# ViV99/slam-experiments

Measured on AMD Instinct MI355X. Metric: descriptor pairs/sec BF-Hamming knn=2 @64kx64k, higher is better.
Workload: dtype u32

## Files before the change

### include/slamhip.h

```cpp
#ifndef SLAMHIP_H
#define SLAMHIP_H

#include <stdint.h>

#ifdef __cplusplus
extern "C" {
#endif

typedef struct slam_ctx slam_ctx;

#define SLAM_API __attribute__((visibility("default")))

enum slam_status {
    SLAM_OK = 0,
    SLAM_ERR_INVALID = -1,
    SLAM_ERR_HIP = -2,
    SLAM_ERR_NO_DEVICE = -3,
    SLAM_ERR_RCCL = -4,
    SLAM_ERR_STATE = -5,
    SLAM_ERR_BUSY = -6
};

#define SLAM_DESC_BYTES 32
#define SLAM_MAX_TRAIN_PER_PASS (1 << 23)
#define SLAM_NO_MATCH_IDX (-1)
#define SLAM_NO_MATCH_DIST 2147483647

SLAM_API const char* slam_last_error(void);
SLAM_API const char* slam_version(void);
SLAM_API int slam_device_count(int* count);
SLAM_API int slam_ctx_create(int device, slam_ctx** out);
SLAM_API int slam_ctx_destroy(slam_ctx* ctx);
SLAM_API int slam_ctx_device(slam_ctx* ctx, int* device);
SLAM_API int slam_sync(slam_ctx* ctx);
SLAM_API int slam_ctx_block_bytes(slam_ctx* ctx, int64_t* h_bytes, int count);
SLAM_API int slam_ctx_block_fill(slam_ctx* ctx, int block, int byte);

SLAM_API int slam_malloc(slam_ctx* ctx, uint64_t bytes, void** d_ptr);
SLAM_API int slam_free(slam_ctx* ctx, void* d_ptr);
SLAM_API int slam_memset(slam_ctx* ctx, void* d_ptr, int value, uint64_t bytes);
SLAM_API int slam_copy(slam_ctx* ctx, void* d_dst, const void* d_src, uint64_t bytes);
SLAM_API int slam_upload(slam_ctx* ctx, void* d_dst, const void* h_src, uint64_t bytes);
SLAM_API int slam_download(slam_ctx* ctx, void* h_dst, const void* d_src, uint64_t bytes);

SLAM_API int slam_timer_start(slam_ctx* ctx);
SLAM_API int slam_timer_stop(slam_ctx* ctx, float* ms);
SLAM_API int slam_prof_enable(slam_ctx* ctx, int on);
SLAM_API int slam_prof_read(slam_ctx* ctx, int64_t* launches, double* total_ms);

SLAM_API int slam_bf_knn2_u256(slam_ctx* ctx, const void* d_query, int64_t N,
                      const void* d_train, int64_t M, int64_t train_base,
                      int32_t* d_idx, int32_t* d_dist);

#define SLAM_BF_BATCH_MAX 32
typedef struct slam_bf_search {
    const void* d_query;
    int64_t N;
    const void* d_train;
    int64_t M;
    int64_t train_base;
    int32_t* d_idx;
    int32_t* d_dist;
} slam_bf_search;
SLAM_API int slam_bf_knn2_batch_u256(slam_ctx* ctx, int64_t B, const slam_bf_search* h_searches);

SLAM_API int slam_bf_merge_top2(slam_ctx* ctx, const int32_t* d_idx_parts,
                       const int32_t* d_dist_parts, int64_t G, int64_t N,
                       int32_t* d_idx, int32_t* d_dist);

SLAM_API int slam_bf_knn2_u256_host(slam_ctx* ctx, const uint8_t* h_query, int64_t N,
                           const uint8_t* h_train, int64_t M,
                           int32_t* h_idx, int32_t* h_dist);

#define SLAM_BF_KNN_MAX 32
SLAM_API int slam_bf_knn_u256(slam_ctx* ctx, const void* d_query, int64_t N, const void* d_train, int64_t M,
                              int64_t train_base, int K, int32_t* d_idx, int32_t* d_dist);
SLAM_API int slam_bf_knn_u256_host(slam_ctx* ctx, const uint8_t* h_query, int64_t N, const uint8_t* h_train, int64_t M,
                                   int K, int32_t* h_idx, int32_t* h_dist);
SLAM_API int slam_bf_merge_topk(slam_ctx* ctx, const int32_t* d_idx_parts, const int32_t* d_dist_parts, int64_t G,
                                int64_t N, int K, int32_t* d_idx, int32_t* d_dist);
SLAM_API int slam_bf_topk_plan_describe(int num_cu, int64_t N, int64_t M, int K, int32_t* h_plan);

SLAM_API int slam_bf_radius_u256(slam_ctx* ctx, const void* d_query, int64_t N, const void* d_train, int64_t M,
                                 float max_distance, int64_t train_base, int64_t* d_offsets, int64_t capacity,
                                 int32_t* d_idx, int32_t* d_dist, int64_t* h_total);
SLAM_API int slam_bf_radius_u256_host(slam_ctx* ctx, const uint8_t* h_query, int64_t N, const uint8_t* h_train, int64_t M,
                                      float max_distance, int64_t* h_offsets, int64_t capacity, int32_t* h_idx,
                                      int32_t* h_dist, int64_t* h_total);
SLAM_API int slam_bf_radius_threshold(float max_distance);
SLAM_API int slam_bf_radius_plan_describe(int num_cu, int64_t N, int64_t M, int32_t* h_plan);

SLAM_API int slam_bf_window_knn_u256(slam_ctx* ctx, const void* d_query, int64_t N, const void* d_train, int64_t M,
                                     const float* d_query_xy, const float* d_train_xy, const float* d_radius, float radius,
                                     int k, int64_t cells, int32_t* d_idx, int32_t* d_dist);
SLAM_API int slam_bf_window_knn_u256_host(slam_ctx* ctx, const uint8_t* h_query, int64_t N, const uint8_t* h_train, int64_t M,
                                          const float* h_query_xy, const float* h_train_xy, const float* h_radius,
                                          float radius, int k, int64_t cells, int32_t* h_idx, int32_t* h_dist);
SLAM_API int slam_bf_window_plan_describe(int num_cu, int64_t N, int64_t M, int64_t cells, int64_t* h_plan);

#define SLAM_BF_KNOBS 10
SLAM_API int slam_bf_set_tuning(slam_ctx* ctx, const int32_t* h_knobs, int count);
SLAM_API int slam_bf_plan_info(slam_ctx* ctx, int64_t N, int64_t M, int32_t* h_plan);
SLAM_API int slam_bf_plan_describe(int num_cu, const int32_t* h_knobs, int count, int64_t N, int64_t M, int64_t qb_all,
                                   int rows_on_host, int32_t* h_plan, int32_t* h_tbl, int64_t tbl_cap, int64_t* tbl_len);
SLAM_API int slam_bf_set_engine(slam_ctx* ctx, int engine);
SLAM_API int slam_bf_mx_plan_describe(int num_cu, int64_t N, int64_t M, int32_t* h_plan, int32_t* h_tbl, int64_t tbl_cap,
                                      int64_t* tbl_len);
SLAM_API int slam_bf_mx_tile_describe(int engine, int64_t N, int64_t M, int32_t* h_tile);
SLAM_API int slam_bf_reset_state(slam_ctx* ctx);
SLAM_API int slam_bf_state_dirty(slam_ctx* ctx, int64_t* h_words);

SLAM_API int slam_bf_knn2_select_u256(slam_ctx* ctx, const void* d_query, int64_t N, const void* d_train, int64_t M,
                                      int64_t train_base, int32_t* d_idx, int32_t* d_dist, int mode, double param,
                                      uint8_t* d_keep, int64_t* h_count);

SLAM_API int slam_bf_match_filter(slam_ctx* ctx, const int32_t* d_idx, const int32_t* d_dist,
                         int64_t N, int mode, double param,
                         uint8_t* d_keep, int64_t* h_count, int32_t* h_min_dist);

SLAM_API int slam_bf_cross_check(slam_ctx* ctx, const int32_t* d_fwd_idx, const int32_t* d_fwd_dist, int64_t N,
                        const int32_t* d_rev_idx, int64_t M, int32_t* d_out_idx, int32_t* d_out_dist,
                        int64_t* h_count);

SLAM_API int slam_bf_split_index(slam_ctx* ctx, const int32_t* d_global_idx, int64_t count, const int32_t* d_offsets,
                                 int64_t images, int32_t* d_img_idx, int32_t* d_train_idx);

SLAM_API int slam_reproj_rj_f64(slam_ctx* ctx, const double* d_poses, int64_t K,
                       const double* d_points, int64_t L,
                       const int32_t* d_obs_pose, const int32_t* d_obs_point,
                       const double* d_meas, int64_t O,
                       double fx, double fy, double cx, double cy,
                       double* d_e, double* d_Jpose, double* d_Jpoint);

SLAM_API int slam_index_errors(slam_ctx* ctx, int64_t* count);

SLAM_API int slam_pose_normal_eq_f64(slam_ctx* ctx, const double* d_pose,
                            const double* d_points, const double* d_meas,
                            const uint8_t* d_active, int64_t O,
                            double fx, double fy, double cx, double cy,
                            double huber_delta,
                            double* d_H, double* d_b, double* d_chi2);

SLAM_API int slam_pose_optimize_f64(slam_ctx* ctx, const double* d_pose_in, const double* d_points,
                                    const double* d_meas, int64_t O, double fx, double fy, double cx, double cy,
                                    int rounds, int iterations, double chi2_threshold, double huber_delta,
                                    double* d_pose_out, uint8_t* d_inlier, double* d_chi2, int32_t* d_stats);

SLAM_API int slam_pose_optimize_batch_f64(slam_ctx* ctx, int64_t B, const double* d_pose_in, const double* d_points,
                                          const double* d_meas, const int32_t* d_offsets, int64_t O_total, double fx,
                                          double fy, double cx, double cy, int rounds, int iterations,
                                          double chi2_threshold, double huber_delta, double* d_pose_out,
                                          uint8_t* d_inlier, double* d_chi2, int32_t* d_stats);


SLAM_API int slam_tv_fivepoint_f64(slam_ctx* ctx, int64_t S, const double* d_x1, const double* d_x2, double* d_E,
                                   int32_t* d_nroots);

SLAM_API int slam_tv_essential_ransac_f64(slam_ctx* ctx, int64_t B, const int32_t* d_offsets, const double* d_px1,
                                          const double* d_px2, int64_t M, double fx, double fy, double cx, double cy,
                                          int H, double threshold_px, uint64_t seed, double* d_E, uint8_t* d_inlier,
                                          int32_t* d_stats);

SLAM_API int slam_tv_recover_pose_f64(slam_ctx* ctx, int64_t B, const int32_t* d_offsets, const double* d_px1,
                                      const double* d_px2, int64_t M, double fx, double fy, double cx, double cy,
                                      const double* d_E, const uint8_t* d_inlier_in, double distance_thresh,
                                      double* d_pose, uint8_t* d_inlier_out, int32_t* d_stats);

SLAM_API int slam_tv_triangulate_f64(slam_ctx* ctx, int64_t N, const double* d_P1, const double* d_P2,
                                     const double* d_x1, const double* d_x2, double* d_X, double* d_w);


SLAM_API int slam_pnp_p3p_f64(slam_ctx* ctx, int64_t S, const double* d_X, const double* d_x, double* d_pose,
                              int32_t* d_nsol);

SLAM_API int slam_pnp_ransac_f64(slam_ctx* ctx, int64_t B, const int32_t* d_offsets, const double* d_X,
                                 const double* d_px, int64_t M, double fx, double fy, double cx, double cy, int H,
                                 double threshold_px, uint64_t seed, double* d_pose, uint8_t* d_inlier,
                                 int32_t* d_stats);


SLAM_API int slam_hg_fourpoint_f64(slam_ctx* ctx, int64_t S, const double* d_p1, const double* d_p2, double* d_H,
                                   int32_t* d_ok);

SLAM_API int slam_hg_ransac_f64(slam_ctx* ctx, int64_t B, const int32_t* d_offsets, const double* d_px1,
                                const double* d_px2, int64_t M, int H, double threshold_px, uint64_t seed, double* d_H,
                                uint8_t* d_inlier, int32_t* d_stats);

SLAM_API int slam_hg_decompose_f64(slam_ctx* ctx, int64_t B, const int32_t* d_offsets, const double* d_px1,
                                   const double* d_px2, int64_t M, double fx, double fy, double cx, double cy,
                                   const double* d_H, const uint8_t* d_inlier_in, double distance_thresh,
                                   double* d_pose_all, double* d_normal_all, int32_t* d_count, double* d_pose,
                                   double* d_sv, uint8_t* d_inlier_out, int32_t* d_stats);

SLAM_API int slam_hg_model_score_f64(slam_ctx* ctx, int64_t B, const int32_t* d_offsets, const double* d_px1,
                                     const double* d_px2, int64_t M, double fx, double fy, double cx, double cy,
                                     const double* d_H, const double* d_E, double sigma, int64_t* d_score,
                                     double* d_ratio);


SLAM_API int slam_sim3_threepoint_f64(slam_ctx* ctx, int64_t S, const double* d_X1, const double* d_X2, int fix_scale,
                                      double* d_model, int32_t* d_ok);

SLAM_API int slam_sim3_ransac_f64(slam_ctx* ctx, int64_t B, const int32_t* d_offsets, const double* d_X1,
                                  const double* d_X2, int64_t M, const double* d_sigma2, double fx, double fy, double cx,
                                  double cy, int H, double chi2_gate, int fix_scale, uint64_t seed, double* d_model,
                                  uint8_t* d_inlier, int32_t* d_stats);

SLAM_API int slam_sim3_refit_f64(slam_ctx* ctx, int64_t B, const int32_t* d_offsets, const double* d_X1,
                                 const double* d_X2, int64_t M, const uint8_t* d_mask, int fix_scale, double* d_model,
                                 int32_t* d_stats);

#define SLAM_ORB_MAX_LEVELS 16
#define SLAM_ORB_MAX_SIDE 8192
#define SLAM_ORB_MAX_BATCH 65535
#define SLAM_ORB_MAX_FEATURES 65536
#define SLAM_ORB_TABLE_BYTES 32768

SLAM_API int slam_orb_workspace(int64_t B, int64_t H, int64_t W, int L, const int32_t* h_level_w, const int32_t* h_level_h,
                                int64_t n_max, uint64_t* bytes, uint64_t* h_layout);

SLAM_API int slam_orb_extract_u8(slam_ctx* ctx, const uint8_t* d_images, int64_t B, int64_t H, int64_t W, const uint8_t* d_mask,
                                 int mask_batched, int L, const int32_t* h_level_w, const int32_t* h_level_h,
                                 const int32_t* h_quota, int fast_threshold, const int8_t* d_table, void* d_workspace,
                                 uint64_t workspace_bytes, int32_t* d_count, int32_t* d_kp, int64_t* d_resp, uint8_t* d_desc);

SLAM_API int slam_orb_extract_u8_host(slam_ctx* ctx, const uint8_t* h_images, int64_t B, int64_t H, int64_t W,
                                      const uint8_t* h_mask, int mask_batched, int L, const int32_t* h_level_w,
                                      const int32_t* h_level_h, const int32_t* h_quota, int fast_threshold,
                                      const int8_t* h_table, int32_t* h_count, int32_t* h_kp, int64_t* h_resp, uint8_t* h_desc);

SLAM_API int slam_bf_match_host(slam_ctx* ctx, const uint8_t* h_query, int64_t N, const uint8_t* h_train,
                                const void* d_train, int64_t M, void* d_query_keep, int mode, double param,
                                int32_t* h_query_idx, int32_t* h_train_idx, float* h_distance, int64_t* h_count);
SLAM_API int slam_io_counters(slam_ctx* ctx, uint64_t* h2d_bytes, uint64_t* d2h_bytes);
SLAM_API int slam_pose_optimize_host_f64(slam_ctx* ctx, const double* h_pose_in, const double* h_points,
                                         const double* h_meas, int64_t O, double fx, double fy, double cx,
                                         double cy, int rounds, int iterations, double chi2_threshold,
                                         double huber_delta, double* h_pose_out, uint8_t* h_inlier,
                                         double* h_chi2, int32_t* h_stats);

#define SLAM_BA_REC 73
SLAM_API int slam_ba_reduce_f64(slam_ctx* ctx, const double* d_poses, int64_t K, const double* d_points,
                                int64_t L, const int32_t* d_obs_pose, const int32_t* d_obs_point,
                                const double* d_meas, int64_t O, const int32_t* d_pt_ptr, const int32_t* d_pt_obs,
                                const int32_t* d_ps_ptr, const int32_t* d_ps_obs, const int32_t* d_lookup,
                                double fx, double fy, double cx, double cy, double huber_delta, double lambda,
                                double* d_rec, double* d_E, double* d_bl, double* d_Hpp, double* d_bp,
                                double* d_ybl, double* d_cost, double* d_W, double* d_hll_diag);
SLAM_API int slam_ba_cost_f64(slam_ctx* ctx, const double* d_poses, int64_t K, const double* d_points,
                              const int32_t* d_obs_point, const double* d_meas, const int32_t* d_ps_ptr,
                              const int32_t* d_ps_obs, double fx, double fy, double cx, double cy,
                              double huber_delta, double* d_cost);
SLAM_API int slam_ba_backsub_f64(slam_ctx* ctx, int64_t L, const int32_t* d_pt_ptr, const int32_t* d_pt_obs,
                                 const int32_t* d_obs_pose, const double* d_rec, const double* d_E,
                                 const double* d_bl, const double* d_dp, double* d_dl);

#define SLAM_BA_LM_MAX_FREE 16
#define SLAM_BA_LM_MAX_OBS (1 << 17)
SLAM_API int slam_ba_optimize_workspace(int64_t K, int64_t L, int64_t O, uint64_t* bytes);
SLAM_API int slam_ba_optimize_shape(int64_t K, int64_t O, int64_t n_free, int32_t* blocks, int32_t* slices);
SLAM_API int slam_ba_optimize_f64(slam_ctx* ctx, int64_t K, int64_t L, int64_t O, const int32_t* d_obs_pose,
                                  const int32_t* d_obs_point, const double* d_meas, const int32_t* d_pt_ptr,
                                  const int32_t* d_pt_obs, const int32_t* d_ps_ptr, const int32_t* d_ps_obs,
                                  const int32_t* d_free_poses, int64_t n_free, double fx, double fy, double cx, double cy,
                                  double huber_delta, int iterations, double* d_poses2, double* d_points2, void* d_work,
                                  uint64_t work_bytes, double* d_stats);
SLAM_API int slam_ba_optimize_host_f64(slam_ctx* ctx, int64_t K, int64_t L, int64_t O, const double* h_poses,
                                       const double* h_points, const int32_t* h_obs_pose, const int32_t* h_obs_point,
                                       const double* h_meas, const uint8_t* h_pose_fixed, double fx, double fy, double cx,
                                       double cy, double huber_delta, int iterations, double* h_poses_out,
                                       double* h_points_out, double* h_stats);

#define SLAM_PG_MAX_VERTICES (1 << 24)
#define SLAM_PG_MAX_EDGES (1 << 25)
#define SLAM_PG_STATUS_INDEX 1
#define SLAM_PG_STATUS_ANGLE 2
#define SLAM_PG_STATUS_PRECOND 4
#define SLAM_PG_STATUS_BREAKDOWN 8
#define SLAM_PG_STATUS_NONFINITE 16
SLAM_API int slam_pg_workspace(int64_t V, int64_t E, uint64_t* bytes);
SLAM_API int slam_pg_plan(int64_t V, int64_t E, int32_t* plan);
SLAM_API int slam_pg_linearize_f64(slam_ctx* ctx, int64_t V, int64_t E, const double* d_poses, const int32_t* d_edges,
                                   const double* d_meas, const double* d_info, const int32_t* d_vtx_ptr,
                                   const int32_t* d_vtx_adj, double huber_delta, double* d_cost, double* d_grad,
                                   double* d_Hdiag, double* d_W, int32_t* h_status);
SLAM_API int slam_pg_hmul_f64(slam_ctx* ctx, int64_t V, int64_t E, const int32_t* d_edges, const int32_t* d_vtx_ptr,
                              const int32_t* d_vtx_adj, const uint8_t* d_fixed, const double* d_Hdiag, const double* d_W,
                              double lambda, const double* d_x, double* d_y);
SLAM_API int slam_pg_pcg_f64(slam_ctx* ctx, int64_t V, int64_t E, const int32_t* d_edges, const int32_t* d_vtx_ptr,
                             const int32_t* d_vtx_adj, const uint8_t* d_fixed, const double* d_Hdiag, const double* d_W,
                             const double* d_b, double lambda, double tol, int max_iter, double* d_x, double* h_stats);
SLAM_API int slam_pg_optimize_f64(slam_ctx* ctx, int64_t V, int64_t E, const double* d_poses, const int32_t* d_edges,
                                  const double* d_meas, const double* d_info, const uint8_t* d_fixed, int64_t n_fixed,
                                  const int32_t* d_vtx_ptr, const int32_t* d_vtx_adj, int iterations, double huber_delta,
                                  double pcg_tol, int pcg_max_iter, double* d_poses_out, double* h_stats);
SLAM_API int slam_pg_optimize_host_f64(slam_ctx* ctx, int64_t V, int64_t E, const double* h_poses, const int32_t* h_edges,
                                       const double* h_meas, const double* h_info, const uint8_t* h_fixed, int iterations,
                                       double huber_delta, double pcg_tol, int pcg_max_iter, double* h_poses_out,
                                       double* h_stats);

#define SLAM_S3G_MAX_VERTICES (1 << 24)
#define SLAM_S3G_MAX_EDGES (1 << 25)
#define SLAM_S3G_STATUS_INDEX 1
#define SLAM_S3G_STATUS_ANGLE 2
#define SLAM_S3G_STATUS_PRECOND 4
#define SLAM_S3G_STATUS_BREAKDOWN 8
#define SLAM_S3G_STATUS_NONFINITE 16
#define SLAM_S3G_STATUS_SCALE 32
SLAM_API int slam_s3g_workspace(int64_t V, int64_t E, uint64_t* bytes);
SLAM_API int slam_s3g_plan(int64_t V, int64_t E, int32_t* plan);
SLAM_API int slam_s3g_linearize_f64(slam_ctx* ctx, int64_t V, int64_t E, const double* d_sims, const int32_t* d_edges,
                                    const double* d_meas, const double* d_info, const int32_t* d_vtx_ptr,
                                    const int32_t* d_vtx_adj, double huber_delta, double* d_cost, double* d_grad,
                                    double* d_Hdiag, double* d_W, int32_t* h_status);
SLAM_API int slam_s3g_hmul_f64(slam_ctx* ctx, int64_t V, int64_t E, const int32_t* d_edges, const int32_t* d_vtx_ptr,
                               const int32_t* d_vtx_adj, const uint8_t* d_fixed, const double* d_Hdiag, const double* d_W,
                               double lambda, const double* d_x, double* d_y);
SLAM_API int slam_s3g_pcg_f64(slam_ctx* ctx, int64_t V, int64_t E, const int32_t* d_edges, const int32_t* d_vtx_ptr,
                              const int32_t* d_vtx_adj, const uint8_t* d_fixed, const double* d_Hdiag, const double* d_W,
                              const double* d_b, double lambda, double tol, int max_iter, double* d_x, double* h_stats);
SLAM_API int slam_s3g_optimize_f64(slam_ctx* ctx, int64_t V, int64_t E, const double* d_sims, const int32_t* d_edges,
                                   const double* d_meas, const double* d_info, const uint8_t* d_fixed, int64_t n_fixed,
                                   const int32_t* d_vtx_ptr, const int32_t* d_vtx_adj, int iterations, double huber_delta,
                                   double pcg_tol, int pcg_max_iter, int fix_scale, double* d_sims_out, double* h_stats);
SLAM_API int slam_s3g_optimize_host_f64(slam_ctx* ctx, int64_t V, int64_t E, const double* h_sims, const int32_t* h_edges,
                                        const double* h_meas, const double* h_info, const uint8_t* h_fixed, int iterations,
                                        double huber_delta, double pcg_tol, int pcg_max_iter, int fix_scale,
                                        double* h_sims_out, double* h_stats);

#define SLAM_BAS_MAX_POINTS (1 << 28)
#define SLAM_BAS_MAX_OBS (1 << 28)
#define SLAM_BAS_MAX_PAIRS (1 << 30)
SLAM_API int slam_bas_workspace(int64_t K, int64_t L, int64_t O, int64_t E, int64_t P, uint64_t* bytes);
SLAM_API int slam_bas_plan(int64_t K, int64_t L, int64_t O, int64_t E, int64_t P, int32_t* plan);
SLAM_API int slam_bas_linearize_f64(slam_ctx* ctx, int64_t K, int64_t L, int64_t O, const double* d_poses, const double* d_points,
                                    const int32_t* d_obs_pose, const int32_t* d_obs_point, const double* d_meas,
                                    const int32_t* d_pt_ptr, const int32_t* d_pt_obs, const int32_t* d_ps_ptr,
                                    const int32_t* d_ps_obs, const uint8_t* d_fixed, double fx, double fy, double cx, double cy,
                                    double huber_delta, double* d_Hpl, double* d_Hll, double* d_bl, double* d_Hpp, double* d_bp,
                                    double* d_cost, double* d_scal);
SLAM_API int slam_bas_cost_f64(slam_ctx* ctx, int64_t K, int64_t L, int64_t O, const double* d_poses, const double* d_points,
                               const int32_t* d_obs_pose, const int32_t* d_obs_point, const double* d_meas,
                               const int32_t* d_ps_ptr, const int32_t* d_ps_obs, double fx, double fy, double cx, double cy,
                               double huber_delta, double* d_cost, double* d_total);
SLAM_API int slam_bas_reduce_f64(slam_ctx* ctx, int64_t K, int64_t L, int64_t O, int64_t E, int64_t P, const int32_t* d_obs_point,
                                 const int32_t* d_pt_ptr, const int32_t* d_ps_ptr, const int32_t* d_ps_obs,
                                 const int32_t* d_pair_ptr, const int32_t* d_pair_a, const int32_t* d_pair_b, const double* d_Hpl,
                                 const double* d_Hll, const double* d_bl, const double* d_Hpp, const double* d_bp, double lambda,
                                 double* d_E, double* d_Ebl, double* d_Hdiag, double* d_W, double* d_b);
SLAM_API int slam_bas_backsub_f64(slam_ctx* ctx, int64_t K, int64_t L, int64_t O, const int32_t* d_pt_ptr, const int32_t* d_pt_obs,
                                  const int32_t* d_obs_pose, const double* d_Hpl, const double* d_E, const double* d_bl,
                                  const double* d_dp, double* d_dl);
SLAM_API int slam_bas_candidate_f64(slam_ctx* ctx, int64_t K, int64_t L, const uint8_t* d_fixed, const double* d_poses,
                                    const double* d_points, const double* d_dp, const double* d_dl, const double* d_bp,
                                    const double* d_bl, double lambda, double* d_poses_out, double* d_points_out, double* d_part,
                                    double* d_denominator);

SLAM_API int slam_bow_limits(int32_t* h_limits);
SLAM_API int slam_bow_transform(slam_ctx* ctx, const void* d_desc, int64_t n, const void* d_node_desc, const int32_t* d_child,
                                const int32_t* d_word_of_node, int64_t n_nodes, int depth, int levels_up, int lanes,
                                int32_t* d_words, int32_t* d_nodes);
SLAM_API int slam_bow_vectors(slam_ctx* ctx, const int32_t* d_words_in, const int64_t* d_offsets, int64_t B, int64_t n,
                              const double* d_idf, int64_t n_words, void* d_ws, uint64_t ws_bytes, int64_t* d_out_offsets,
                              int32_t* d_out_words, double* d_out_values, uint32_t* d_out_q);
SLAM_API int slam_bow_vectors_workspace(int64_t B, int64_t n, uint64_t* h_bytes);
SLAM_API int slam_bow_group_keys(slam_ctx* ctx, const int32_t* d_keys, int64_t n, int64_t n_keys, int32_t* d_key_off,
                                 int32_t* d_cursor, int32_t* d_perm);
SLAM_API int slam_bow_index_build(slam_ctx* ctx, const int32_t* d_words, const int32_t* d_entry, const uint32_t* d_q, int64_t T,
                                  int64_t n_words, int32_t* d_word_off, int32_t* d_cursor, int32_t* d_perm, void* d_postings);
SLAM_API int slam_bow_query(slam_ctx* ctx, const int64_t* d_q_offsets, const int32_t* d_q_words, const uint32_t* d_q_q, int64_t Q,
                            const int32_t* d_word_off, const void* d_postings, int64_t n_words, int64_t E, int64_t max_id,
                            int max_results, int32_t* d_ids, uint32_t* d_s_int, int32_t* d_common, uint32_t* d_dense_s,
                            int32_t* d_dense_common);
SLAM_API int slam_bow_train_seed(slam_ctx* ctx, const void* d_desc, int64_t n, const int32_t* d_row_node, int64_t F, int k,
                                 void* d_cent, int32_t* d_cent_count, void* d_ws, uint64_t ws_bytes);
SLAM_API int slam_bow_train_seed_workspace(int64_t n, int64_t F, uint64_t* h_bytes);
SLAM_API int slam_bow_train_step(slam_ctx* ctx, const void* d_desc, int64_t n, const int32_t* d_row_node, int64_t F, int k,
                                 void* d_cent, const int32_t* d_cent_count, int32_t* d_assign, const int32_t* d_perm,
                                 int64_t n_live, uint32_t* d_bits, uint32_t* d_rows_of, uint32_t* d_changed, int update,
                                 int64_t* h_changed);
SLAM_API int slam_bow_train_descend(slam_ctx* ctx, int32_t* d_row_node, const int32_t* d_assign, int64_t n, int64_t F, int k,
                                    uint32_t* d_own, const int32_t* d_next_of);

#define SLAM_BOW_MATCH_ROWS_MAX 8192
#define SLAM_BOW_MATCH_PAIRS_MAX 4096
SLAM_API int slam_bow_match_limits(int32_t* h_limits);
SLAM_API int slam_bow_match_plan_describe(int64_t B, int64_t n, int64_t* h_plan);
SLAM_API int slam_bow_match_group(slam_ctx* ctx, const void* d_desc, const int32_t* d_nodes, const int64_t* h_offsets, int64_t B,
                                  void* d_desc_sorted, int32_t* d_nodes_sorted, int32_t* d_order, int32_t* d_inverse);
typedef struct slam_bow_groups {
    const void* d_desc;
    const int32_t* d_nodes;
    const int32_t* d_order;
    const int32_t* d_inverse;
    const uint8_t* d_bins;
    const int64_t* h_offsets;
    int64_t B;
} slam_bow_groups;
SLAM_API int slam_bow_match_top2(slam_ctx* ctx, const slam_bow_groups* g1, const slam_bow_groups* g2, const int32_t* h_pairs, int64_t P,
                                 int scan_order, int32_t* d_idx, int32_t* d_dist);
SLAM_API int slam_bow_match_search(slam_ctx* ctx, const slam_bow_groups* g1, const slam_bow_groups* g2, const int32_t* h_pairs, int64_t P,
                                   int th_low, double ratio, int scan_order, int32_t* d_matches12, int32_t* d_count, int32_t* d_idx,
                                   int32_t* d_dist);

#define SLAM_PROJ_MATCH_ROWS_MAX 8192
#define SLAM_PROJ_MATCH_PAIRS_MAX 4096
#define SLAM_PROJ_MATCH_LEVELS_MAX 16
SLAM_API int slam_proj_match_limits(int32_t* h_limits);
SLAM_API int slam_proj_match_plan_describe(int64_t B, int64_t P, int64_t n, int64_t* h_plan);
SLAM_API int slam_proj_match_grid(slam_ctx* ctx, const void* d_desc, const float* d_xy, const int32_t* d_level, const uint8_t* d_taken,
                                  const int64_t* h_offsets, int64_t B, int W, int H, int cell, int32_t* d_cells, void* d_desc_sorted,
                                  int32_t* d_cells_sorted, int32_t* d_order, int32_t* d_inverse, float* d_xy_sorted,
                                  int32_t* d_meta_sorted);
typedef struct slam_proj_frames {
    const void* d_desc;
    const int32_t* d_cells;
    const int32_t* d_order;
    const float* d_xy;
    const int32_t* d_meta;
    const int32_t* d_level;
    const uint8_t* d_bins;
    const int64_t* h_offsets;
    int64_t B;
    int32_t W, H, cell, pad;
} slam_proj_frames;
typedef struct slam_proj_points {
    const double* d_xyz;
    const void* d_desc;
    const double* d_range;
    const double* d_normal;
    const int32_t* d_level;
    const uint8_t* d_bins;
    const int64_t* h_offsets;
    int64_t B;
} slam_proj_points;
typedef struct slam_proj_params {
    double fx, fy, cx, cy;
    double min_x, max_x, min_y, max_y;
    double cos2_limit, ratio;
    const double* h_scale;
    const double* h_scale2;
    int32_t n_levels, th_high, level_rule, lo, hi, pad;
} slam_proj_params;
SLAM_API int slam_proj_match_project(slam_ctx* ctx, const slam_proj_points* points, const int32_t* h_sets, const double* h_poses,
                                     const double* h_centres, const double* h_th, int64_t P, const slam_proj_params* params,
                                     int32_t* d_status, double* d_u, double* d_v, int32_t* d_lp);
SLAM_API int slam_proj_match_search(slam_ctx* ctx, const slam_proj_points* points, const slam_proj_frames* frames, const int32_t* h_pairs,
                                    const double* h_poses, const double* h_centres, const double* h_th, int64_t P,
                                    const slam_proj_params* params, int32_t* d_matches12, int32_t* d_count, int32_t* d_status, double* d_u,
                                    double* d_v, int32_t* d_lp, int32_t* d_idx, int32_t* d_dist);

#define SLAM_TRI_MATCH_ROWS_MAX 8192
#define SLAM_TRI_MATCH_PAIRS_MAX 4096
#define SLAM_TRI_MATCH_LEVELS_MAX 16
SLAM_API int slam_tri_match_limits(int32_t* h_limits);
SLAM_API int slam_tri_match_plan_describe(int64_t P, int64_t n, int64_t* h_plan);
typedef struct slam_tri_views {
    const float* d_xy;
    const int32_t* d_level;
    const uint8_t* d_taken;
} slam_tri_views;
typedef struct slam_tri_params {
    double fx, fy, cx, cy;
    double chi2, epipole_r2;
    double cos_max, chi2_px, ratio_factor;
    const double* h_scale;
    const double* h_sigma2;
    int32_t n_levels, th_low;
} slam_tri_params;
SLAM_API int slam_tri_match_search(slam_ctx* ctx, const slam_bow_groups* g1, const slam_bow_groups* g2, const slam_tri_views* views1,
                                   const slam_tri_views* views2, const int32_t* h_pairs, int64_t P, const double* h_F,
                                   const double* h_epipole, const slam_tri_params* params, int scan_order, int32_t* d_matches12,
                                   int32_t* d_count, int32_t* d_idx, int32_t* d_dist);
SLAM_API int slam_tri_match_triangulate(slam_ctx* ctx, const int64_t* h_offsets1, int64_t B1, const int64_t* h_offsets2, int64_t B2,
                                        const slam_tri_views* views1, const slam_tri_views* views2, const int32_t* h_pairs, int64_t P,
                                        const int32_t* d_matches12, const double* h_T1, const double* h_T2, const double* h_O1,
                                        const double* h_O2, const slam_tri_params* params, double* d_X, double* d_normal,
                                        double* d_range, int32_t* d_status, int32_t* d_created);

#define SLAM_FUSE_OBS_MAX 256
SLAM_API int slam_fuse_limits(int32_t* h_limits);
typedef struct slam_fuse_params {
    double m_lo2, m_hi2, chi2;
    int32_t th_low, pad;
} slam_fuse_params;
SLAM_API int slam_fuse_search(slam_ctx* ctx, const slam_proj_points* points, const int32_t* d_id, const slam_proj_frames* frames,
                              const int32_t* d_point, const int64_t* h_obs_offsets, const int64_t* d_obs_offsets, const int32_t* d_obs,
                              int64_t M, const int32_t* h_pairs, const double* h_poses, const double* h_centres, const double* h_th, int64_t P,
                              const slam_proj_params* params, const slam_fuse_params* fuse, int32_t* d_row, int32_t* d_dist,
                              int32_t* d_status, int32_t* d_other, int32_t* d_count, double* d_u, double* d_v, int32_t* d_lp);
SLAM_API int slam_fuse_refresh(slam_ctx* ctx, const double* d_xyz, const int64_t* h_obs_offsets, const int32_t* d_obs, int64_t M,
                               const int32_t* h_select, int64_t K, const void* d_desc, const int32_t* d_inverse, const int32_t* d_level,
                               const int64_t* h_frame_offsets, int64_t B, const double* d_centres, const int32_t* d_ref, const double* h_scale,
                               int n_levels, int32_t* d_best, void* d_desc_out, double* d_normal, double* d_range);

SLAM_API int slam_covis_limits(int32_t* h_limits);
SLAM_API int slam_covis_plan(int64_t K, int64_t L, int64_t O, int64_t P, int32_t* h_plan);
SLAM_API int slam_covis_workspace(int64_t K, int64_t L, int64_t O, int64_t P, uint64_t* h_bytes);
SLAM_API int slam_covis_count(slam_ctx* ctx, int64_t K, int64_t L, int64_t O, const int32_t* d_obs_pose, const int32_t* d_obs_point,
                              const uint8_t* d_fixed, void* d_count_ws, int64_t* h_scalars);
SLAM_API int slam_covis_pairs(slam_ctx* ctx, int64_t K, int64_t L, int64_t O, int64_t P, const void* d_count_ws, void* d_pair_ws,
                              int32_t* d_pair_a, int32_t* d_pair_b, int64_t* h_edges);
SLAM_API int slam_covis_edges(slam_ctx* ctx, int64_t K, int64_t P, int64_t E, const void* d_pair_ws, int32_t* d_edges, int32_t* d_weights,
                              int32_t* d_pair_ptr);
SLAM_API int slam_covis_rows(slam_ctx* ctx, int64_t M, int64_t nnz, const int64_t* d_offsets, const int32_t* d_obs, int32_t* d_obs_pose,
                             int32_t* d_obs_point);

#define SLAM_COMM_ID_BYTES 128
SLAM_API int slam_comm_version(int* version);
SLAM_API int slam_comm_unique_id(void* h_id );
SLAM_API int slam_comm_init(slam_ctx* ctx, int nranks, int rank, const void* h_id);
SLAM_API int slam_comm_destroy(slam_ctx* ctx);
SLAM_API int slam_comm_allgather(slam_ctx* ctx, const void* d_send, void* d_recv, uint64_t bytes_per_rank);
SLAM_API int slam_comm_broadcast(slam_ctx* ctx, void* d_buf, uint64_t bytes, int root);
SLAM_API int slam_comm_allgather_overlapped(slam_ctx* ctx, const void* d_send, void* d_recv, uint64_t bytes_per_rank,
                                            int buffer_id);
SLAM_API int slam_comm_wait_buffer(slam_ctx* ctx, int buffer_id);

#define SLAM_P2P_HANDLE_BYTES 64
SLAM_API int slam_p2p_export(slam_ctx* ctx, void* d_ptr, void* h_handle );
SLAM_API int slam_p2p_open(slam_ctx* ctx, const void* h_handle, void** d_peer_ptr);
SLAM_API int slam_p2p_close(slam_ctx* ctx, void* d_peer_ptr);
SLAM_API int slam_p2p_allgather_overlapped(slam_ctx* ctx, const void* d_send, uint64_t bytes_per_rank, int rank,
                                           void* const* h_peer_bufs, int nranks, int buffer_id);

#ifdef __cplusplus
}
#endif
#endif
```

### slam-experiments_amd/csrc/bf_mx.hip

```cpp
#include "internal.h"
#include <vector>
#include <atomic>
#include <type_traits>

#include "bf_common.h"
#include "bf_mx_common.h"

#define SLAM_MX_UNROLL 4

#ifdef SLAM_MX_PROBE
__device__ unsigned long long* g_mx_probe = nullptr;
extern "C" __attribute__((visibility("default"))) int slam_exp_set_mx_probe(void* p) {
    return (int)hipMemcpyToSymbol(HIP_SYMBOL(g_mx_probe), &p, sizeof(p));
}
#endif

typedef float mx_v4f __attribute__((ext_vector_type(4)));

__device__ __forceinline__ mx_v4f mx_dot(uint4 a, uint4 b, mx_v4f c) {
    const mx_v8i av = {(int)a.x, (int)a.y, (int)a.z, (int)a.w, 0, 0, 0, 0};
    const mx_v8i bv = {(int)b.x, (int)b.y, (int)b.z, (int)b.w, 0, 0, 0, 0};
    return __builtin_amdgcn_mfma_scale_f32_16x16x128_f8f6f4(av, bv, c, 4, 4, 0, 127, 0, 127);
}

__device__ __forceinline__ u32 mx_pick(const u32 (&v)[4], int i) {
    return i == 0 ? v[0] : (i == 1 ? v[1] : (i == 2 ? v[2] : v[3]));
}

__global__ __launch_bounds__(256) __attribute__((amdgpu_waves_per_eu(4, 4))) void bf_top2_mx_kernel(const uint4* __restrict__ q, int N, const uint4* __restrict__ t,
                                                         const int* __restrict__ tbl, bf_state st, int train_base,
                                                         int2* __restrict__ out_idx, int2* __restrict__ out_dist,
                                                         uint4* __restrict__ keep, int nchunks, bf_select sel) {
    __shared__ uint4 tile[2][SLAM_MX_STAGE * 8];
    __shared__ u32 s_ticket, s_last;
    const int tid = threadIdx.x;
    const int lane = tid & 63, wave = tid >> 6;
    const int kg = lane >> 4, col = lane & 15;
#ifdef SLAM_MX_PROBE
    unsigned long long pacc[8] = {0, 0, 0, 0, 0, 0, 0, 0}, plast = __builtin_readcyclecounter();
#endif
    const u32 lanek = (u32)(4 * kg - (1 << SLAM_KEY_IDX_BITS));
    const int bx = ((int)blockIdx.x + (int)blockIdx.y) % (int)gridDim.x;
    auto lane_query = [&]() -> int {
        int v = tid;
        asm volatile("" : "+v"(v));
        return bx * 256 + v;
    };

    uint4 qb[4][2];
    const u32* qw = (const u32*)q;
#pragma unroll
    for (int tt = 0; tt < 4; tt++) {
        int qi = bx * 256 + wave * 64 + tt * 16 + col;
        qi = qi < N ? qi : N - 1;
#pragma unroll
        for (int h = 0; h < 2; h++) qb[tt][h] = mx_expand(qw[(size_t)qi * 8 + h * 4 + kg]);
    }
    if (const int qbase = lane_query(); keep && blockIdx.y == 0 && qbase < N) {
        keep[2 * (size_t)qbase] = q[2 * (size_t)qbase];
        keep[2 * (size_t)qbase + 1] = q[2 * (size_t)qbase + 1];
    }

    u32 b1[4], b2[4];
    mx_v4f cth[4];
    auto set_threshold = [&](int tt, u32 x) {
        const float c = (float)(2 * (int)x - 258);
        cth[tt] = mx_v4f{c, c, c, c};
    };
    auto threshold_x = [&](int tt) -> u32 { return (u32)((int)cth[tt][0] + 258) >> 1; };
#pragma unroll
    for (int tt = 0; tt < 4; tt++) {
        b1[tt] = b2[tt] = SLAM_KEY_NONE;
        set_threshold(tt, SLAM_KEY_NONE >> SLAM_KEY_IDX_BITS);
    }
    auto unite_tile = [&](int tt, u32& u1, u32& u2) {
        u1 = b1[tt];
        u2 = b2[tt];
#pragma unroll
        for (int off = 16; off <= 32; off <<= 1) {
            const u32 c1 = (u32)__shfl_xor((int)u1, off, 64), c2 = (u32)__shfl_xor((int)u2, off, 64);
            mx_unite(u1, u2, c1, c2);
        }
    };
    auto unite_lanes = [&](u32 (&u1)[4], u32 (&u2)[4]) {
#pragma unroll
        for (int tt = 0; tt < 4; tt++) unite_tile(tt, u1[tt], u2[tt]);
    };
    u32 gkey = SLAM_BOUND_IDLE, pend[1] = {0u};
    auto exchange = [&](int c0) {
        u32 u1[4], u2[4];
        unite_lanes(u1, u2);
        if (const int qbase = lane_query(); qbase < N) {
            const u32 own = mx_pick(u2, kg);
            asm volatile("" ::"v"(pend[0]));
            const u32 g = __hip_atomic_load(&st.bound[qbase], __ATOMIC_RELAXED, __HIP_MEMORY_SCOPE_AGENT);
            if (own < g && own < SLAM_MX_BOUND_LIMIT) pend[0] = atomicMin(&st.bound[qbase], own);
            gkey = g;
        }
#pragma unroll
        for (int tt = 0; tt < 4; tt++) {
            const u32 g = (u32)__shfl((int)gkey, tt * 16 + col, 64);
            const u32 gx = mx_bound_x(g, c0);
            set_threshold(tt, min(threshold_x(tt), min(gx, u2[tt] >> SLAM_KEY_IDX_BITS)));
        }
    };

    const int srow = tid >> 1, sh = tid & 1;
    auto load_stage = [&](int s, int c1) -> uint4 {
        const uint4* ts = t + 2 * (size_t)s;
        if (s + SLAM_MX_STAGE <= c1) return ts[(u32)tid];
        return s + srow < c1 ? ts[(u32)tid] : make_uint4(0, 0, 0, 0);
    };
    const u32 fill = 0x22222222u;
    auto expand = [&](u32 v) -> uint4 { return mx_expand_op(v, fill); };
    uint4* const dst0 = tile[0] + (srow >> 4) * 128 + sh * 64 + (srow & 15);
    auto store_stage = [&](int b, uint4 v) {
        uint4* dst = dst0 + b * (SLAM_MX_STAGE * 8);
        dst[0] = expand(v.x);
        dst[16] = expand(v.y);
        dst[32] = expand(v.z);
        dst[48] = expand(v.w);
    };

    u32* const cursor = st.cursor + (size_t)(4 * bx) * SLAM_CURSOR_STRIDE;
    if (tid == 0) s_ticket = __hip_atomic_fetch_add(cursor, 1u, __ATOMIC_RELAXED, __HIP_MEMORY_SCOPE_AGENT);
    __syncthreads();
    int ci = __builtin_amdgcn_readfirstlane((int)s_ticket);
    int scanned = 0;
    MX_STAMP(0);
    while (ci < nchunks) {
        const int c0 = tbl[ci], c1 = tbl[ci + 1];
        const uint4 first = load_stage(c0, c1);
        exchange(c0);
        store_stage(0, first);
        __syncthreads();
        MX_STAMP(1);
        int buf = 0;
        for (int s0 = c0; s0 < c1; s0 += SLAM_MX_STAGE) {
            const int s1 = s0 + SLAM_MX_STAGE;
            const bool more = s1 < c1;
            if (!more && tid == 0) s_ticket = __hip_atomic_fetch_add(cursor, 1u, __ATOMIC_RELAXED, __HIP_MEMORY_SCOPE_AGENT);
            MX_STAMP(7);
            const int ng = __builtin_amdgcn_readfirstlane(min(SLAM_MX_STAGE / 16, (c1 - s0 + 15) >> 4));
            const uint4* tp = tile[buf];
            auto dots0 = [&](const uint4& a, mx_v4f (&acc)[4]) {
#pragma unroll
                for (int tt = 0; tt < 4; tt++) acc[tt] = mx_dot(a, qb[tt][0], cth[tt]);
            };
            auto fold = [&](int g, mx_v4f (&acc)[4], auto rag) {
                int p[4];
#pragma unroll
                for (int tt = 0; tt < 4; tt++)
                    p[tt] = max(max(__float_as_int(acc[tt][0]), __float_as_int(acc[tt][1])), __float_as_int(acc[tt][2]));
                int m = max(max(p[0], __float_as_int(acc[0][3])), p[1]);
                m = max(max(m, __float_as_int(acc[1][3])), p[2]);
                m = max(max(m, __float_as_int(acc[2][3])), p[3]);
                m = max(m, __float_as_int(acc[3][3]));
                if (__builtin_expect(__ballot(m >= 0) != 0ull, 0)) {
                    MX_STAMP(2);
                    int row0 = s0 + g * 16;
                    asm("" : "+s"(row0));
                    const u32 rowk = (u32)row0 + lanek;
#pragma unroll
                    for (int tt = 0; tt < 4; tt++) {
                        if (__ballot(max(p[tt], __float_as_int(acc[tt][3])) >= 0) == 0ull) continue;
                        const u32 xt = threshold_x(tt);
                        const u32 base = (xt << SLAM_KEY_IDX_BITS) + rowk;
#pragma unroll
                        for (int r = 0; r < 4; r++) {
                            if (__ballot(__float_as_int(acc[tt][r]) >= 0) == 0ull) continue;
                            u32 key = base + (u32)r + ((u32)(int)(-acc[tt][r]) << (SLAM_KEY_IDX_BITS - 1));
                            if constexpr (decltype(rag)::value)
                                key = (int)rowk + r < c1 - (1 << SLAM_KEY_IDX_BITS) ? key : SLAM_KEY_NONE;
                            b2[tt] = umed3(b1[tt], b2[tt], key);
                            b1[tt] = min(b1[tt], key);
                        }
                        set_threshold(tt, min(xt, b2[tt] >> SLAM_KEY_IDX_BITS));
                    }
                    MX_STAMP(3);
                }
            };
            auto group = [&](int g, auto rag) {
                const uint4 a0 = tp[g * 128 + lane], a1 = tp[g * 128 + 64 + lane];
                mx_v4f acc[4];
                dots0(a0, acc);
#pragma unroll
                for (int tt = 0; tt < 4; tt++) acc[tt] = mx_dot(a1, qb[tt][1], acc[tt]);
                fold(g, acc, rag);
            };
            auto trip = [&](int g0, auto ngc, auto shadow) {
                constexpr int NG = decltype(ngc)::value;
                constexpr bool SH = decltype(shadow)::value;
                const uint4* ap = tp + g0 * 128 + lane;
                uint4* const dst = dst0 + (buf ^ 1) * (SLAM_MX_STAGE * 8);
                u32 nx[4] = {0, 0, 0, 0};
                if (SH) {
                    const uint4 x = (t + 2 * (size_t)s1)[2 * min(srow, c1 - 1 - s1) + sh];
                    nx[0] = x.x; nx[1] = x.y; nx[2] = x.z; nx[3] = x.w;
                }
                uint4 a0 = ap[0], a1 = ap[64];
#pragma unroll
                for (int k = 0; k < NG; k++) {
                    uint4 a0n = a0, a1n = a1;
                    mx_v4f acc[4];
                    if (k + 1 < NG) a0n = ap[(k + 1) * 128];
                    const u32 v = nx[SH && k >= NG - 4 ? k - (NG - 4) : 0];
                    __builtin_amdgcn_sched_barrier(0);
                    dots0(a0, acc);
                    __builtin_amdgcn_sched_barrier(0);
                    if (SH && k >= NG - 4) {
                        const int j = k - (NG - 4);
                        uint4 e;
                        acc[0] = mx_dot(a1, qb[0][1], acc[0]);
                        __builtin_amdgcn_sched_barrier(0);
                        asm volatile("v_lshlrev_b32 %0, 3, %1\n\tv_and_or_b32 %0, %0, %2, %3" : "=v"(e.x) : "v"(v), "s"(0x88888888u), "v"(fill));
                        asm volatile("v_lshlrev_b32 %0, 2, %1" : "=v"(e.y) : "v"(v));
                        __builtin_amdgcn_sched_barrier(0);
                        acc[1] = mx_dot(a1, qb[1][1], acc[1]);
                        __builtin_amdgcn_sched_barrier(0);
                        asm volatile("v_and_or_b32 %0, %1, %2, %3" : "=v"(e.y) : "v"(e.y), "s"(0x88888888u), "v"(fill));
                        asm volatile("v_lshlrev_b32 %0, 1, %1\n\tv_and_or_b32 %0, %0, %2, %3" : "=v"(e.z) : "v"(v), "s"(0x88888888u), "v"(fill));
                        __builtin_amdgcn_sched_barrier(0);
                        acc[2] = mx_dot(a1, qb[2][1], acc[2]);
                        __builtin_amdgcn_sched_barrier(0);
                        asm volatile("v_and_or_b32 %0, %1, %2, %3" : "=v"(e.w) : "v"(v), "s"(0x88888888u), "v"(fill));
                        dst[16 * j] = e;
                        if (k + 1 < NG) a1n = ap[(k + 1) * 128 + 64];
                        __builtin_amdgcn_sched_barrier(0);
                        acc[3] = mx_dot(a1, qb[3][1], acc[3]);
                    } else {
                        if (k + 1 < NG) a1n = ap[(k + 1) * 128 + 64];
                        __builtin_amdgcn_sched_barrier(0);
#pragma unroll
                        for (int tt = 0; tt < 4; tt++) acc[tt] = mx_dot(a1, qb[tt][1], acc[tt]);
                    }
                    fold(g0 + k, acc, std::false_type{});
                    __builtin_amdgcn_sched_barrier(0);
                    a0 = a0n;
                    a1 = a1n;
                }
            };
            const int nwhole = __builtin_amdgcn_readfirstlane(min(SLAM_MX_STAGE / 16, (c1 - s0) >> 4));
            int g = 0;
            if (more) {
                trip(0, std::integral_constant<int, SLAM_MX_STAGE / 16>{}, std::true_type{});
                g = SLAM_MX_STAGE / 16;
            }
            for (; g + SLAM_MX_UNROLL <= nwhole; g += SLAM_MX_UNROLL) trip(g, std::integral_constant<int, SLAM_MX_UNROLL>{}, std::false_type{});
            for (; g < ng; g++) group(g, std::true_type{});
            MX_STAMP(2);
            scanned += min(s1, c1) - s0;
            if (more && scanned < 32 * SLAM_MX_STAGE && (SLAM_MX_EARLY >> (scanned / SLAM_MX_STAGE) & 1u)) exchange(s1);
            MX_STAMP(4);
            __syncthreads();
            MX_STAMP(5);
            buf ^= 1;
        }
        ci = __builtin_amdgcn_readfirstlane((int)s_ticket);
    }

    u32 u1[4], u2[4];
    unite_lanes(u1, u2);
    const u32 f1[1] = {mx_pick(u1, kg)}, f2[1] = {mx_pick(u2, kg)};
    const u32 gk[1] = {gkey < SLAM_MX_BOUND_LIMIT ? gkey >> SLAM_KEY_IDX_BITS : SLAM_BOUND_IDLE};
    bf_top2_epilogue<1, true>(st, bx, tid, lane, lane_query(), false, false, f1, f2, gk, pend, N, (int)gridDim.y, train_base, out_idx,
                              out_dist, sel, s_last);
#ifdef SLAM_MX_PROBE
    MX_STAMP(6);
    if (g_mx_probe && lane == 0) {
        unsigned long long* o = g_mx_probe + ((size_t)(blockIdx.y * gridDim.x + blockIdx.x) * 4 + wave) * 8;
        for (int i = 0; i < 8; i++) o[i] = pacc[i];
    }
#endif
}


struct bf_mx_plan {
    int qblocks;
    int workers;
    int chunk;
    int S;
    int tail;
};

static bf_mx_plan make_mx_plan_core(int num_cu, int resident, int64_t N, int64_t M, std::vector<int>* tbl) {
    bf_mx_plan p;
    p.qblocks = (int)((N + 255) / 256);
    int64_t W = (int64_t)num_cu * resident / p.qblocks;
    if (W < 1) W = 1;
    if (W > 256) W = 256;
    const int64_t c = M / W >= 8192 ? 1024 : 256;
    std::vector<int>& b = *tbl;
    b.clear();
    b.push_back(0);
    int shrinking = 0;
    for (int64_t at = 0; at < M;) {
        int64_t len = c;
        const int64_t g = (M - at) / (2 * W) / SLAM_MX_STAGE * SLAM_MX_STAGE;
        if (g < len) { len = g < SLAM_MX_STAGE ? SLAM_MX_STAGE : g; shrinking++; }
        at = at + len < M ? at + len : M;
        b.push_back((int)at);
    }
    p.chunk = (int)c;
    p.S = (int)b.size() - 1;
    p.tail = shrinking;
    p.workers = (int)(W < p.S ? W : p.S);
    return p;
}

static bool bf_mx_auto(int64_t N, int64_t M) {
    return (N >= 8192 && M >= 16384) || (N >= 3000 && M >= 40000) || (N >= 1000 && M >= 65536) || (N >= 500 && M >= 200000);
}

extern "C" int slam_bf_mx_plan_describe(int num_cu, int64_t N, int64_t M, int32_t* h_plan, int32_t* h_tbl, int64_t tbl_cap,
                                        int64_t* tbl_len) {
    SLAM_REQUIRE(num_cu >= 1 && num_cu <= 4096, "num_cu out of range");
    SLAM_REQUIRE(N >= 1 && M >= 1 && M <= SLAM_MAX_TRAIN_PER_PASS && N <= (1ll << 30), "bad sizes");
    SLAM_REQUIRE(h_plan && tbl_len && (h_tbl || tbl_cap == 0) && tbl_cap >= 0, "slam_bf_mx_plan_describe: null argument");
    std::vector<int> tbl;
    const bf_mx_plan p = make_mx_plan_core(num_cu, SLAM_MX_RESIDENT, N, M, &tbl);
    h_plan[0] = p.qblocks; h_plan[1] = p.workers; h_plan[2] = p.chunk; h_plan[3] = p.S;
    h_plan[4] = p.tail; h_plan[5] = SLAM_MX_STAGE; h_plan[6] = SLAM_MX_RESIDENT; h_plan[7] = bf_mx_auto(N, M) ? 1 : 0;
    *tbl_len = (int64_t)tbl.size();
    for (int64_t i = 0; i < (int64_t)tbl.size() && i < tbl_cap; i++) h_tbl[i] = tbl[(size_t)i];
    return SLAM_OK;
}

static bool bf_mx32_auto(int64_t N, int64_t M) {
    return N <= 131072 && M <= 200000;
}

extern "C" int slam_bf_mx_tile_describe(int engine, int64_t N, int64_t M, int32_t* h_tile) {
    SLAM_REQUIRE(h_tile, "slam_bf_mx_tile_describe: null argument");
    SLAM_REQUIRE(engine == 0 || engine == 2 || engine == 3, "engine must be 0 (auto), 2 or 3");
    SLAM_REQUIRE(N >= 1 && M >= 1, "bad sizes");
    *h_tile = engine == 3 || (engine == 0 && bf_mx32_auto(N, M)) ? 32 : 16;
    return SLAM_OK;
}

extern "C" int slam_bf_set_engine(slam_ctx* ctx, int engine) {
    SLAM_REQUIRE(ctx, "slam_bf_set_engine: null ctx");
    SLAM_REQUIRE(engine >= 0 && engine <= 3,
                 "engine must be 0 (auto), 1 (VALU), 2 (16x16 matrix-core kernel where eligible) or 3 (32x32 matrix-core kernel where eligible)");
    std::lock_guard<std::mutex> g(ctx->mu);
    ctx->bf_engine = engine;
    return SLAM_OK;
}

bool bf_mx_route(slam_ctx* ctx, int64_t N, int64_t M, bool rows_on_host) {
    std::lock_guard<std::mutex> g(ctx->mu);
    if (ctx->bf_engine == 1 || rows_on_host) return false;
    for (int i = 0; i < SLAM_BF_KNOBS; i++)
        if (ctx->bf_knob[i]) return false;
    return ctx->bf_engine == 2 || ctx->bf_engine == 3 || bf_mx_auto(N, M);
}

int bf_mx_pass(slam_ctx* ctx, const void* d_query, int64_t N, const void* d_train, int64_t M, int64_t train_base, int32_t* d_idx,
               int32_t* d_dist, void* d_keep, const bf_select& sel, int* qblocks_out) {
    int num_cu, engine;
    {
        std::lock_guard<std::mutex> g(ctx->mu);
        num_cu = ctx->num_cu;
        engine = ctx->bf_engine;
    }
    const bool wide = engine == 3 || (engine == 0 && bf_mx32_auto(N, M));
    const auto kernel = wide ? bf_top2_mx32_kernel : bf_top2_mx_kernel;
    static std::atomic<int> occ_once[2] = {{0}, {0}};
    int occ = occ_once[wide].load(std::memory_order_relaxed);
    if (!occ) {
        int o = 0;
        SLAM_HIP(hipOccupancyMaxActiveBlocksPerMultiprocessor(&o, kernel, 256, 0));
        occ = o > 0 ? o : SLAM_MX_RESIDENT;
        occ_once[wide].store(occ, std::memory_order_relaxed);
    }
    std::vector<int> tbl;
    const bf_mx_plan p = make_mx_plan_core(num_cu, occ, N, M, &tbl);
    bf_state st;
    if (int rc = bf_state_get(ctx, N, &st)) return rc;
    const int* d_tbl = nullptr;
    if (int rc = bf_table_get(ctx, tbl, &d_tbl)) return rc;
    if (qblocks_out) *qblocks_out = p.qblocks;
    SLAM_HIP(hipGetLastError());
    if (int rc = slam_prof_begin(ctx)) return rc;
    kernel<<<dim3(p.qblocks, p.workers), dim3(256), 0, ctx->stream>>>(
        (const uint4*)d_query, (int)N, (const uint4*)d_train, d_tbl, st, (int)train_base, (int2*)d_idx, (int2*)d_dist,
        (uint4*)d_keep, p.S, sel);
    if (int rc = slam_prof_end(ctx)) return rc;
    const hipError_t e = hipGetLastError();
    if (e != hipSuccess) {
        (void)bf_state_reset(ctx);
        return slam_set_error(SLAM_ERR_HIP, "top-2 MX kernel launch failed: %s", hipGetErrorString(e));
    }
    return SLAM_OK;
}
```

### slam-experiments_amd/csrc/bf_mx32.hip

```cpp
#include "internal.h"
#include <type_traits>

#include "bf_common.h"
#include "bf_mx_common.h"

typedef float mx_v16f __attribute__((ext_vector_type(16)));

#ifdef SLAM_MX_PROBE
__device__ unsigned long long* g_mx32_probe = nullptr;
extern "C" __attribute__((visibility("default"))) int slam_exp_set_mx32_probe(void* p) {
    return (int)hipMemcpyToSymbol(HIP_SYMBOL(g_mx32_probe), &p, sizeof(p));
}
#endif

__device__ __forceinline__ mx_v16f mx32_dot(uint4 a, uint4 b, mx_v16f c) {
    const mx_v8i av = {(int)a.x, (int)a.y, (int)a.z, (int)a.w, 0, 0, 0, 0};
    const mx_v8i bv = {(int)b.x, (int)b.y, (int)b.z, (int)b.w, 0, 0, 0, 0};
    return __builtin_amdgcn_mfma_scale_f32_32x32x64_f8f6f4(av, bv, c, 4, 4, 0, 0, 0, 0);
}

#define MX32_GROUP 32
#define MX32_GROUPS (SLAM_MX_STAGE / MX32_GROUP)

__global__ __launch_bounds__(256) __attribute__((amdgpu_waves_per_eu(4, 4))) void bf_top2_mx32_kernel(
    const uint4* __restrict__ q, int N, const uint4* __restrict__ t, const int* __restrict__ tbl, bf_state st, int train_base,
    int2* __restrict__ out_idx, int2* __restrict__ out_dist, uint4* __restrict__ keep, int nchunks, bf_select sel) {
    __shared__ uint4 tile[2][SLAM_MX_STAGE * 8];
    __shared__ u32 s_ticket, s_last;
    const int tid = threadIdx.x;
    const int lane = tid & 63, wave = tid >> 6;
    const int hk = lane >> 5, col = lane & 31;
#ifdef SLAM_MX_PROBE
    unsigned long long pacc[8] = {0, 0, 0, 0, 0, 0, 0, 0}, plast = __builtin_readcyclecounter();
#endif
    const int bx = ((int)blockIdx.x + (int)blockIdx.y) % (int)gridDim.x;
    auto lane_query = [&]() -> int {
        int v = tid;
        asm volatile("" : "+v"(v));
        return bx * 256 + v;
    };

    uint4 qb[2][4];
    const u32* qw = (const u32*)q;
#pragma unroll
    for (int tt = 0; tt < 2; tt++) {
        int qi = bx * 256 + wave * 64 + tt * 32 + col;
        qi = qi < N ? qi : N - 1;
#pragma unroll
        for (int kq = 0; kq < 4; kq++) qb[tt][kq] = mx_expand(qw[(size_t)qi * 8 + kq * 2 + hk]);
    }
    if (const int qbase = lane_query(); keep && blockIdx.y == 0 && qbase < N) {
        keep[2 * (size_t)qbase] = q[2 * (size_t)qbase];
        keep[2 * (size_t)qbase + 1] = q[2 * (size_t)qbase + 1];
    }

    u32 b1[2], b2[2], xs[2];
    int thr[2];
    auto set_threshold = [&](int tt, u32 x) {
        xs[tt] = x;
        thr[tt] = x > 129u ? (int)0x80000000u : __float_as_int((float)(258 - 2 * (int)x));
    };
#pragma unroll
    for (int tt = 0; tt < 2; tt++) {
        b1[tt] = b2[tt] = SLAM_KEY_NONE;
        set_threshold(tt, SLAM_KEY_NONE >> SLAM_KEY_IDX_BITS);
    }
    auto unite_tile = [&](int tt, u32& u1, u32& u2) {
        u1 = b1[tt];
        u2 = b2[tt];
        const u32 c1 = (u32)__shfl_xor((int)u1, 32, 64), c2 = (u32)__shfl_xor((int)u2, 32, 64);
        mx_unite(u1, u2, c1, c2);
    };
    u32 gkey = SLAM_BOUND_IDLE, pend[1] = {0u};
    auto exchange = [&](int c0) {
        u32 u1[2], u2[2];
#pragma unroll
        for (int tt = 0; tt < 2; tt++) unite_tile(tt, u1[tt], u2[tt]);
        if (const int qbase = lane_query(); qbase < N) {
            const u32 own = hk ? u2[1] : u2[0];
            asm volatile("" ::"v"(pend[0]));
            const u32 g = __hip_atomic_load(&st.bound[qbase], __ATOMIC_RELAXED, __HIP_MEMORY_SCOPE_AGENT);
            if (own < g && own < SLAM_MX_BOUND_LIMIT) pend[0] = atomicMin(&st.bound[qbase], own);
            gkey = g;
        }
#pragma unroll
        for (int tt = 0; tt < 2; tt++) {
            const u32 g = (u32)__shfl((int)gkey, tt * 32 + col, 64);
            set_threshold(tt, min(xs[tt], min(mx_bound_x(g, c0), u2[tt] >> SLAM_KEY_IDX_BITS)));
        }
    };

    const int srow = tid >> 1, sh = tid & 1;
    auto load_stage = [&](int s, int c1) -> uint4 {
        const uint4* ts = t + 2 * (size_t)s;
        if (s + SLAM_MX_STAGE <= c1) return ts[(u32)tid];
        return s + srow < c1 ? ts[(u32)tid] : make_uint4(0, 0, 0, 0);
    };
    const u32 fill = 0x22222222u;
    uint4* const dst0 = tile[0] + (srow >> 5) * 256 + sh * 128 + (srow & 31);
    auto store_word = [&](uint4* dst, int j, u32 v) { dst[(j >> 1) * 64 + (j & 1) * 32] = mx_expand_op(v, fill); };
    auto store_stage = [&](int b, uint4 v) {
        uint4* dst = dst0 + b * (SLAM_MX_STAGE * 8);
        store_word(dst, 0, v.x);
        store_word(dst, 1, v.y);
        store_word(dst, 2, v.z);
        store_word(dst, 3, v.w);
    };

    u32* const cursor = st.cursor + (size_t)(4 * bx) * SLAM_CURSOR_STRIDE;
    if (tid == 0) s_ticket = __hip_atomic_fetch_add(cursor, 1u, __ATOMIC_RELAXED, __HIP_MEMORY_SCOPE_AGENT);
    __syncthreads();
    int ci = __builtin_amdgcn_readfirstlane((int)s_ticket);
    int scanned = 0;
    MX_STAMP(0);
    while (ci < nchunks) {
        const int c0 = tbl[ci], c1 = tbl[ci + 1];
        const uint4 first = load_stage(c0, c1);
        exchange(c0);
        store_stage(0, first);
        __syncthreads();
        MX_STAMP(1);
        int buf = 0;
        for (int s0 = c0; s0 < c1; s0 += SLAM_MX_STAGE) {
            const int s1 = s0 + SLAM_MX_STAGE;
            const bool more = s1 < c1;
            if (!more && tid == 0) s_ticket = __hip_atomic_fetch_add(cursor, 1u, __ATOMIC_RELAXED, __HIP_MEMORY_SCOPE_AGENT);
            MX_STAMP(7);
            const uint4* tp = tile[buf];
            auto fold_tile = [&](int tt, int g, const mx_v16f& acc, auto rag) {
                int p = max(max(__float_as_int(acc[0]), __float_as_int(acc[1])), __float_as_int(acc[2]));
#pragma unroll
                for (int i = 3; i < 15; i += 2) p = max(max(p, __float_as_int(acc[i])), __float_as_int(acc[i + 1]));
                const int m = max(p, __float_as_int(acc[15]));
                if (__builtin_expect(__ballot(m >= thr[tt]) == 0ull, 1)) return;
                MX_STAMP(2);
                int row0 = s0 + g * MX32_GROUP;
                asm("" : "+s"(row0));
                const u32 rowk = (u32)row0 + (u32)(4 * hk);
                const u32 base = (128u << SLAM_KEY_IDX_BITS) + rowk;
                unsigned long long gate[16];
#pragma unroll
                for (int i = 0; i < 16; i++) gate[i] = __ballot(__float_as_int(acc[i]) >= thr[tt]);
                asm volatile("" ::"s"(gate[0]), "s"(gate[1]), "s"(gate[2]), "s"(gate[3]), "s"(gate[4]), "s"(gate[5]), "s"(gate[6]),
                             "s"(gate[7]), "s"(gate[8]), "s"(gate[9]), "s"(gate[10]), "s"(gate[11]), "s"(gate[12]), "s"(gate[13]),
                             "s"(gate[14]), "s"(gate[15]));
#pragma unroll
                for (int i = 0; i < 16; i++) {
                    if (gate[i] == 0ull) continue;
                    const int off = 8 * (i >> 2) + (i & 3);
                    u32 key = base + (u32)off + ((u32)(int)(-acc[i]) << (SLAM_KEY_IDX_BITS - 1));
                    if constexpr (decltype(rag)::value)
                        key = (int)rowk + off < c1 ? key : SLAM_KEY_NONE;
                    b2[tt] = umed3(b1[tt], b2[tt], key);
                    b1[tt] = min(b1[tt], key);
                }
                set_threshold(tt, min(xs[tt], b2[tt] >> SLAM_KEY_IDX_BITS));
                MX_STAMP(3);
            };
            const mx_v16f zero = {0, 0, 0, 0, 0, 0, 0, 0, 0, 0, 0, 0, 0, 0, 0, 0};
            auto group = [&](int g, auto rag) {
                mx_v16f acc[2];
#pragma unroll
                for (int kq = 0; kq < 4; kq++) {
                    const uint4 a = tp[g * 256 + kq * 64 + lane];
#pragma unroll
                    for (int tt = 0; tt < 2; tt++) acc[tt] = mx32_dot(a, qb[tt][kq], kq ? acc[tt] : zero);
                }
#pragma unroll
                for (int tt = 0; tt < 2; tt++) fold_tile(tt, g, acc[tt], rag);
            };
            auto trip = [&](auto shadow) {
                constexpr bool SH = decltype(shadow)::value;
                const uint4* ap = tp + lane;
                uint4* const dst = dst0 + (buf ^ 1) * (SLAM_MX_STAGE * 8);
                u32 nx[4] = {0, 0, 0, 0};
                if (SH) {
                    const uint4 x = (t + 2 * (size_t)s1)[2 * min(srow, c1 - 1 - s1) + sh];
                    nx[0] = x.x; nx[1] = x.y; nx[2] = x.z; nx[3] = x.w;
                }
                uint4 a[4];
#pragma unroll
                for (int kq = 0; kq < 4; kq++) a[kq] = ap[kq * 64];
                mx_v16f acc[2];
                auto dot = [&](int tt, int kq) {
                    __builtin_amdgcn_sched_barrier(0);
                    acc[tt] = mx32_dot(a[kq], qb[tt][kq], kq ? acc[tt] : zero);
                    __builtin_amdgcn_sched_barrier(0);
                };
#pragma unroll
                for (int k = 0; k < MX32_GROUPS; k++) {
                    auto ahead = [&](int kq) {
                        if (k + 1 < MX32_GROUPS) a[kq] = ap[(k + 1) * 256 + kq * 64];
                        __builtin_amdgcn_sched_barrier(0);
                    };
                    dot(0, 0);
                    dot(0, 1);
                    dot(0, 2);
                    dot(0, 3);
                    if (k) fold_tile(1, k - 1, acc[1], std::false_type{});
                    dot(1, 0);
                    ahead(0);
                    dot(1, 1);
                    ahead(1);
                    if (SH && k >= 1) store_word(dst, k - 1, nx[k - 1]);
                    dot(1, 2);
                    ahead(2);
                    if (SH && k == 3) store_word(dst, 3, nx[3]);
                    dot(1, 3);
                    ahead(3);
                    fold_tile(0, k, acc[0], std::false_type{});
                }
                __builtin_amdgcn_sched_barrier(0);
                fold_tile(1, MX32_GROUPS - 1, acc[1], std::false_type{});
            };
            if (more) {
                trip(std::true_type{});
            } else if (s1 == c1) {
                trip(std::false_type{});
            } else {
                const int ng = __builtin_amdgcn_readfirstlane((c1 - s0 + MX32_GROUP - 1) / MX32_GROUP);
                for (int g = 0; g < ng; g++) group(g, std::true_type{});
            }
            MX_STAMP(2);
            scanned += min(s1, c1) - s0;
            if (more && scanned < 32 * SLAM_MX_STAGE && (SLAM_MX_EARLY >> (scanned / SLAM_MX_STAGE) & 1u)) exchange(s1);
            MX_STAMP(4);
            __syncthreads();
            MX_STAMP(5);
            buf ^= 1;
        }
        ci = __builtin_amdgcn_readfirstlane((int)s_ticket);
    }

    u32 u1[2], u2[2];
#pragma unroll
    for (int tt = 0; tt < 2; tt++) unite_tile(tt, u1[tt], u2[tt]);
    const u32 f1[1] = {hk ? u1[1] : u1[0]}, f2[1] = {hk ? u2[1] : u2[0]};
    const u32 gk[1] = {gkey < SLAM_MX_BOUND_LIMIT ? gkey >> SLAM_KEY_IDX_BITS : SLAM_BOUND_IDLE};
    bf_top2_epilogue<1, true>(st, bx, tid, lane, lane_query(), false, false, f1, f2, gk, pend, N, (int)gridDim.y, train_base, out_idx,
                              out_dist, sel, s_last);
#ifdef SLAM_MX_PROBE
    MX_STAMP(6);
    if (g_mx32_probe && lane == 0) {
        unsigned long long* o = g_mx32_probe + ((size_t)(blockIdx.y * gridDim.x + blockIdx.x) * 4 + wave) * 8;
        for (int i = 0; i < 8; i++) o[i] = pacc[i];
    }
#endif
}
```

### slam-experiments_amd/csrc/bf_mx_common.h

```cpp
#pragma once
#include "internal.h"
#include "bf_common.h"

#define SLAM_MX_STAGE 128
#define SLAM_MX_BOUND_LIMIT 0x7F000000u
#define SLAM_MX_EARLY 0x16u
#define SLAM_MX_RESIDENT 4

#ifdef SLAM_MX_PROBE
#define MX_STAMP(ph) do { const unsigned long long now_ = __builtin_readcyclecounter(); pacc[ph] += now_ - plast; plast = now_; } while (0)
#else
#define MX_STAMP(ph) do {} while (0)
#endif

typedef int mx_v8i __attribute__((ext_vector_type(8)));

__device__ __forceinline__ uint4 mx_expand(u32 x) {
    uint4 r;
    r.x = ((x << 3) & 0x88888888u) | 0x22222222u;
    r.y = ((x << 2) & 0x88888888u) | 0x22222222u;
    r.z = ((x << 1) & 0x88888888u) | 0x22222222u;
    r.w = (x & 0x88888888u) | 0x22222222u;
    return r;
}

__device__ __forceinline__ uint4 mx_expand_op(u32 v, u32 fill) {
    uint4 r;
    asm("v_and_or_b32 %0, %1, %2, %3" : "=v"(r.x) : "v"(v << 3), "s"(0x88888888u), "v"(fill));
    asm("v_and_or_b32 %0, %1, %2, %3" : "=v"(r.y) : "v"(v << 2), "s"(0x88888888u), "v"(fill));
    asm("v_and_or_b32 %0, %1, %2, %3" : "=v"(r.z) : "v"(v << 1), "s"(0x88888888u), "v"(fill));
    asm("v_and_or_b32 %0, %1, %2, %3" : "=v"(r.w) : "v"(v), "s"(0x88888888u), "v"(fill));
    return r;
}

__device__ __forceinline__ void mx_unite(u32& b1, u32& b2, u32 c1, u32 c2) {
    const u32 n2 = min(max(b1, c1), min(b2, c2));
    b1 = min(b1, c1);
    b2 = n2;
}

__device__ __forceinline__ u32 mx_bound_x(u32 g, int c0) {
    return g < SLAM_MX_BOUND_LIMIT ? (g >> SLAM_KEY_IDX_BITS) + ((g & SLAM_KEY_IDX_MASK) < (u32)c0 ? 0u : 1u)
                                   : SLAM_KEY_NONE >> SLAM_KEY_IDX_BITS;
}

__global__ void bf_top2_mx32_kernel(const uint4* __restrict__ q, int N, const uint4* __restrict__ t, const int* __restrict__ tbl,
                                    bf_state st, int train_base, int2* __restrict__ out_idx, int2* __restrict__ out_dist,
                                    uint4* __restrict__ keep, int nchunks, bf_select sel);
```

### slam-experiments_amd/csrc/ctx.hip

```cpp
#include "internal.h"
#include <stdio.h>
#include <string.h>
#include <new>

static thread_local char g_err[512] = "";

int slam_set_error(int code, const char* fmt, ...) {
    va_list ap;
    va_start(ap, fmt);
    vsnprintf(g_err, sizeof(g_err), fmt, ap);
    va_end(ap);
    return code;
}

extern "C" const char* slam_last_error(void) { return g_err; }
extern "C" const char* slam_version(void) { return "slamhip 0.3 (gfx950)"; }

extern "C" int slam_device_count(int* count) {
    SLAM_REQUIRE(count, "slam_device_count: null out pointer");
    int n = 0;
    hipError_t e = hipGetDeviceCount(&n);
    if (e != hipSuccess) {
        *count = 0;
        return slam_set_error(SLAM_ERR_NO_DEVICE, "hipGetDeviceCount: %s", hipGetErrorString(e));
    }
    *count = n;
    return SLAM_OK;
}

extern "C" int slam_ctx_create(int device, slam_ctx** out) {
    SLAM_REQUIRE(out, "slam_ctx_create: null out pointer");
    *out = nullptr;
    int n = 0;
    if (hipGetDeviceCount(&n) != hipSuccess || n == 0)
        return slam_set_error(SLAM_ERR_NO_DEVICE, "no HIP device visible");
    SLAM_REQUIRE(device >= 0 && device < n, "device %d out of range [0,%d)", device, n);
    SLAM_HIP(hipSetDevice(device));
    hipDeviceProp_t prop;
    SLAM_HIP(hipGetDeviceProperties(&prop, device));
    if (strncmp(prop.gcnArchName, "gfx950", 6) != 0)
        return slam_set_error(SLAM_ERR_NO_DEVICE, "device %d is %s, library is built for gfx950 only",
                              device, prop.gcnArchName);
    slam_ctx* c = new (std::nothrow) slam_ctx();
    SLAM_REQUIRE(c, "out of host memory");
    c->device = device;
    c->num_cu = prop.multiProcessorCount;
    hipError_t e = hipStreamCreateWithFlags(&c->stream, hipStreamNonBlocking);
    if (e == hipSuccess) e = hipEventCreate(&c->ev_start);
    if (e == hipSuccess) e = hipEventCreate(&c->ev_stop);
    if (e == hipSuccess) e = hipMalloc(&c->scratch, 4096);
    if (e == hipSuccess) e = hipMemsetAsync(c->scratch, 0, 4096, c->stream);
    if (e == hipSuccess) e = hipStreamSynchronize(c->stream);
    if (e != hipSuccess) {
        delete c;
        return slam_set_error(SLAM_ERR_HIP, "context setup failed: %s", hipGetErrorString(e));
    }
    *out = c;
    return SLAM_OK;
}

extern "C" int slam_ctx_destroy(slam_ctx* ctx) {
    if (!ctx) return SLAM_OK;
    (void)hipSetDevice(ctx->device);
    (void)hipStreamSynchronize(ctx->stream);
    if (ctx->comm) slam_comm_destroy(ctx);
    slam_second_stream_destroy(ctx);
    for (auto& kv : ctx->allocs) (void)hipFree(kv.first);
    if (ctx->workspace) (void)hipFree(ctx->workspace);
    if (ctx->radius_mem) (void)hipFree(ctx->radius_mem);
    if (ctx->scratch) (void)hipFree(ctx->scratch);
    if (ctx->io_dev) (void)hipFree(ctx->io_dev);
    if (ctx->io_host) (void)hipHostFree(ctx->io_host);
    if (ctx->sel_host) (void)hipHostFree(ctx->sel_host);
    for (void* old : ctx->sel_host_old) (void)hipHostFree(old);
    if (ctx->bf_state_mem) (void)hipFree(ctx->bf_state_mem);
    if (ctx->bf_tbl_ready) {
        (void)hipFree(ctx->bf_tbl_dev);
        (void)hipHostFree(ctx->bf_tbl_host);
        for (int i = 0; i < SLAM_BF_TBL_RING; i++) (void)hipEventDestroy(ctx->bf_tbl_ev[i]);
    }
    if (ctx->prof_ev) {
        for (int i = 0; i < 2 * slam_ctx::PROF_MAX; i++) (void)hipEventDestroy(ctx->prof_ev[i]);
        delete[] ctx->prof_ev;
    }
    (void)hipEventDestroy(ctx->ev_start);
    (void)hipEventDestroy(ctx->ev_stop);
    (void)hipStreamDestroy(ctx->stream);
    delete ctx;
    return SLAM_OK;
}

extern "C" int slam_ctx_device(slam_ctx* ctx, int* device) {
    SLAM_REQUIRE(ctx && device, "slam_ctx_device: null argument");
    *device = ctx->device;
    return SLAM_OK;
}

extern "C" int slam_sync(slam_ctx* ctx) {
    SLAM_REQUIRE(ctx, "slam_sync: null ctx");
    SLAM_HIP(hipSetDevice(ctx->device));
    SLAM_HIP(hipStreamSynchronize(ctx->stream));
    if (ctx->comm_stream) SLAM_HIP(hipStreamSynchronize(ctx->comm_stream));
    return SLAM_OK;
}

extern "C" int slam_malloc(slam_ctx* ctx, uint64_t bytes, void** d_ptr) {
    SLAM_REQUIRE(ctx && d_ptr, "slam_malloc: null argument");
    *d_ptr = nullptr;
    SLAM_HIP(hipSetDevice(ctx->device));
    void* p = nullptr;
    SLAM_HIP(hipMalloc(&p, bytes ? bytes : 16));
    std::lock_guard<std::mutex> g(ctx->mu);
    ctx->allocs[p] = bytes;
    *d_ptr = p;
    return SLAM_OK;
}

extern "C" int slam_free(slam_ctx* ctx, void* d_ptr) {
    SLAM_REQUIRE(ctx, "slam_free: null ctx");
    if (!d_ptr) return SLAM_OK;
    {
        std::lock_guard<std::mutex> g(ctx->mu);
        auto it = ctx->allocs.find(d_ptr);
        SLAM_REQUIRE(it != ctx->allocs.end(), "slam_free: pointer %p not owned by this context", d_ptr);
        ctx->allocs.erase(it);
    }
    SLAM_HIP(hipSetDevice(ctx->device));
    SLAM_HIP(hipStreamSynchronize(ctx->stream));
    if (ctx->comm_stream) SLAM_HIP(hipStreamSynchronize(ctx->comm_stream));
    SLAM_HIP(hipFree(d_ptr));
    return SLAM_OK;
}

extern "C" int slam_memset(slam_ctx* ctx, void* d_ptr, int value, uint64_t bytes) {
    SLAM_REQUIRE(ctx && (d_ptr || !bytes), "slam_memset: null argument");
    if (!bytes) return SLAM_OK;
    SLAM_HIP(hipSetDevice(ctx->device));
    SLAM_HIP(hipMemsetAsync(d_ptr, value, bytes, ctx->stream));
    return SLAM_OK;
}

extern "C" int slam_copy(slam_ctx* ctx, void* d_dst, const void* d_src, uint64_t bytes) {
    SLAM_REQUIRE(ctx && ((d_dst && d_src) || !bytes), "slam_copy: null argument");
    if (!bytes) return SLAM_OK;
    SLAM_HIP(hipSetDevice(ctx->device));
    SLAM_HIP(hipMemcpyAsync(d_dst, d_src, bytes, hipMemcpyDeviceToDevice, ctx->stream));
    return SLAM_OK;
}

extern "C" int slam_upload(slam_ctx* ctx, void* d_dst, const void* h_src, uint64_t bytes) {
    SLAM_REQUIRE(ctx && ((d_dst && h_src) || !bytes), "slam_upload: null argument");
    if (!bytes) return SLAM_OK;
    SLAM_HIP(hipSetDevice(ctx->device));
    SLAM_HIP(hipMemcpyAsync(d_dst, h_src, bytes, hipMemcpyHostToDevice, ctx->stream));
    SLAM_HIP(hipStreamSynchronize(ctx->stream));
    return SLAM_OK;
}

extern "C" int slam_download(slam_ctx* ctx, void* h_dst, const void* d_src, uint64_t bytes) {
    SLAM_REQUIRE(ctx && ((h_dst && d_src) || !bytes), "slam_download: null argument");
    if (!bytes) return SLAM_OK;
    SLAM_HIP(hipSetDevice(ctx->device));
    SLAM_HIP(hipMemcpyAsync(h_dst, d_src, bytes, hipMemcpyDeviceToHost, ctx->stream));
    SLAM_HIP(hipStreamSynchronize(ctx->stream));
    return SLAM_OK;
}

int slam_workspace(slam_ctx* ctx, uint64_t bytes, void** out) {
    if (bytes > ctx->workspace_bytes) {
        SLAM_HIP(hipStreamSynchronize(ctx->stream));
        if (ctx->workspace) SLAM_HIP(hipFree(ctx->workspace));
        ctx->workspace = nullptr;
        ctx->workspace_bytes = 0;
        uint64_t want = bytes + (bytes >> 2);
        SLAM_HIP(hipMalloc(&ctx->workspace, want));
        ctx->workspace_bytes = want;
    }
    *out = ctx->workspace;
    return SLAM_OK;
}

int slam_io_arena(slam_ctx* ctx, uint64_t dev_bytes, uint64_t host_bytes, void** dev, void** host) {
    if (dev_bytes > ctx->io_dev_bytes || host_bytes > ctx->io_host_bytes) SLAM_HIP(hipStreamSynchronize(ctx->stream));
    if (dev_bytes > ctx->io_dev_bytes) {
        if (ctx->io_dev) SLAM_HIP(hipFree(ctx->io_dev));
        ctx->io_dev = nullptr;
        ctx->io_dev_bytes = 0;
        const uint64_t want = dev_bytes + (dev_bytes >> 2) + 4096;
        SLAM_HIP(hipMalloc(&ctx->io_dev, want));
        ctx->io_dev_bytes = want;
    }
    if (host_bytes > ctx->io_host_bytes) {
        if (ctx->io_host) SLAM_HIP(hipHostFree(ctx->io_host));
        ctx->io_host = nullptr;
        ctx->io_host_bytes = 0;
        const uint64_t want = host_bytes + (host_bytes >> 2) + 4096;
        SLAM_HIP(hipHostMalloc(&ctx->io_host, want, hipHostMallocDefault));
        ctx->io_host_bytes = want;
    }
    *dev = ctx->io_dev;
    *host = ctx->io_host;
    return SLAM_OK;
}

int slam_launch_check(const char* what) {
    const hipError_t e = hipGetLastError();
    if (e != hipSuccess) return slam_set_error(SLAM_ERR_HIP, "%s launch failed: %s", what, hipGetErrorString(e));
    return SLAM_OK;
}

int slam_occupancy_once(const void* kernel, std::atomic<int>* once, int* out) {
    int occ = once->load(std::memory_order_relaxed);
    if (!occ) {
        int o = 0;
        SLAM_HIP(hipOccupancyMaxActiveBlocksPerMultiprocessor(&o, kernel, 256, 0));
        occ = o > 0 ? o : 1;
        once->store(occ, std::memory_order_relaxed);
    }
    *out = occ;
    return SLAM_OK;
}

bf_chunks bf_chunk_rule(int num_cu, int resident, int64_t N, int64_t rows, int64_t min_chunk, int64_t bytes_per_chunk,
                        int64_t cap_bytes) {
    bf_chunks c;
    c.qblocks = (int)((N + 255) / 256);
    const int64_t slots = (int64_t)(num_cu > 0 ? num_cu : 1) * resident;
    const int64_t qb = c.qblocks > 0 ? c.qblocks : 1;
    int64_t chunks = (slots + qb - 1) / qb;
    const int64_t by_rows = (rows + min_chunk - 1) / min_chunk;
    if (chunks > by_rows) chunks = by_rows;
    const int64_t by_cap = cap_bytes / (bytes_per_chunk > 0 ? bytes_per_chunk : 1);
    if (chunks > by_cap) chunks = by_cap;
    if (chunks < 1) chunks = 1;
    int64_t chunk = (rows + chunks - 1) / chunks;
    chunk = (chunk + 15) / 16 * 16;
    if (chunk < 16) chunk = 16;
    c.chunk = chunk;
    c.chunks = (int)((rows + chunk - 1) / chunk);
    if (c.chunks < 1) c.chunks = 1;
    return c;
}

extern "C" int slam_index_errors(slam_ctx* ctx, int64_t* count) {
    SLAM_REQUIRE(ctx && count, "slam_index_errors: null argument");
    SLAM_HIP(hipSetDevice(ctx->device));
    unsigned int h = 0;
    SLAM_HIP(hipMemcpyAsync(&h, slam_index_error_counter(ctx), sizeof(h), hipMemcpyDeviceToHost, ctx->stream));
    SLAM_HIP(hipMemsetAsync(slam_index_error_counter(ctx), 0, sizeof(h), ctx->stream));
    SLAM_HIP(hipStreamSynchronize(ctx->stream));
    *count = h;
    return SLAM_OK;
}

extern "C" int slam_io_counters(slam_ctx* ctx, uint64_t* h2d_bytes, uint64_t* d2h_bytes) {
    SLAM_REQUIRE(ctx, "slam_io_counters: null ctx");
    std::lock_guard<std::mutex> lk(ctx->call_mu);
    if (h2d_bytes) *h2d_bytes = ctx->io_h2d_bytes;
    if (d2h_bytes) *d2h_bytes = ctx->io_d2h_bytes;
    return SLAM_OK;
}

extern "C" int slam_ctx_block_bytes(slam_ctx* ctx, int64_t* h_bytes, int count) {
    SLAM_REQUIRE(ctx && (h_bytes || count == 0) && count >= 0 && count <= 6, "slam_ctx_block_bytes: bad argument");
    std::lock_guard<std::mutex> lk(ctx->call_mu);
    const int64_t b[6] = {(int64_t)ctx->workspace_bytes, ctx->bf_state_mem ? (int64_t)bf_state_bytes((size_t)ctx->bf_state_rows) : 0,
                          (int64_t)ctx->sel_host_bytes, (int64_t)ctx->io_dev_bytes, (int64_t)ctx->io_host_bytes,
                          (int64_t)ctx->radius_mem_bytes};
    for (int i = 0; i < count; i++) h_bytes[i] = b[i];
    return SLAM_OK;
}

extern "C" int slam_ctx_block_fill(slam_ctx* ctx, int block, int byte) {
    SLAM_REQUIRE(ctx, "slam_ctx_block_fill: null ctx");
    SLAM_REQUIRE(block == 0 || (block >= 3 && block <= 5), "slam_ctx_block_fill: block %d is not a scratch block (0, 3, 4, 5)", block);
    std::lock_guard<std::mutex> lk(ctx->call_mu);
    SLAM_HIP(hipSetDevice(ctx->device));
    SLAM_HIP(hipStreamSynchronize(ctx->stream));
    if (block == 4) {
        if (ctx->io_host) memset(ctx->io_host, byte, ctx->io_host_bytes);
        return SLAM_OK;
    }
    void* p = block == 0 ? ctx->workspace : block == 3 ? ctx->io_dev : ctx->radius_mem;
    const uint64_t n = block == 0 ? ctx->workspace_bytes : block == 3 ? ctx->io_dev_bytes : ctx->radius_mem_bytes;
    if (!p || !n) return SLAM_OK;
    SLAM_HIP(hipMemsetAsync(p, byte, n, ctx->stream));
    SLAM_HIP(hipStreamSynchronize(ctx->stream));
    return SLAM_OK;
}

extern "C" int slam_timer_start(slam_ctx* ctx) {
    SLAM_REQUIRE(ctx, "slam_timer_start: null ctx");
    SLAM_HIP(hipSetDevice(ctx->device));
    SLAM_HIP(hipEventRecord(ctx->ev_start, ctx->stream));
    return SLAM_OK;
}

extern "C" int slam_timer_stop(slam_ctx* ctx, float* ms) {
    SLAM_REQUIRE(ctx && ms, "slam_timer_stop: null argument");
    SLAM_HIP(hipSetDevice(ctx->device));
    SLAM_HIP(hipEventRecord(ctx->ev_stop, ctx->stream));
    SLAM_HIP(hipEventSynchronize(ctx->ev_stop));
    SLAM_HIP(hipEventElapsedTime(ms, ctx->ev_start, ctx->ev_stop));
    return SLAM_OK;
}

extern "C" int slam_prof_enable(slam_ctx* ctx, int on) {
    SLAM_REQUIRE(ctx, "slam_prof_enable: null ctx");
    SLAM_HIP(hipSetDevice(ctx->device));
    if (on && !ctx->prof_ev) {
        ctx->prof_ev = new (std::nothrow) hipEvent_t[2 * slam_ctx::PROF_MAX];
        SLAM_REQUIRE(ctx->prof_ev, "out of host memory");
        for (int i = 0; i < 2 * slam_ctx::PROF_MAX; i++) SLAM_HIP(hipEventCreate(&ctx->prof_ev[i]));
    }
    ctx->prof_on = on ? 1 : 0;
    ctx->prof_n = 0;
    return SLAM_OK;
}

int slam_prof_begin(slam_ctx* ctx) {
    if (!ctx->prof_on || ctx->prof_n >= slam_ctx::PROF_MAX) return SLAM_OK;
    SLAM_HIP(hipEventRecord(ctx->prof_ev[2 * ctx->prof_n], ctx->stream));
    return SLAM_OK;
}

int slam_prof_end(slam_ctx* ctx) {
    if (!ctx->prof_on || ctx->prof_n >= slam_ctx::PROF_MAX) return SLAM_OK;
    SLAM_HIP(hipEventRecord(ctx->prof_ev[2 * ctx->prof_n + 1], ctx->stream));
    ctx->prof_n++;
    return SLAM_OK;
}

extern "C" int slam_prof_read(slam_ctx* ctx, int64_t* launches, double* total_ms) {
    SLAM_REQUIRE(ctx && launches && total_ms, "slam_prof_read: null argument");
    SLAM_HIP(hipSetDevice(ctx->device));
    SLAM_HIP(hipStreamSynchronize(ctx->stream));
    double sum = 0;
    for (int i = 0; i < ctx->prof_n; i++) {
        float ms = 0;
        SLAM_HIP(hipEventElapsedTime(&ms, ctx->prof_ev[2 * i], ctx->prof_ev[2 * i + 1]));
        sum += ms;
    }
    *launches = ctx->prof_n;
    *total_ms = sum;
    ctx->prof_n = 0;
    return SLAM_OK;
}
```

### slam-experiments_amd/csrc/internal.h

```cpp
#pragma once
#include <hip/hip_runtime.h>
#include <stdint.h>
#include <stdarg.h>
#include <string.h>
#include <unordered_map>
#include <atomic>
#include <mutex>
#include <vector>
#include "slamhip.h"

#define SLAM_BF_TBL_RING 8
#define SLAM_BF_TBL_SLOT 4096

struct slam_ctx {
    int device = -1;
    hipStream_t stream = nullptr;
    hipEvent_t ev_start = nullptr, ev_stop = nullptr;
    std::mutex call_mu;
    std::mutex mu;
    std::unordered_map<void*, uint64_t> allocs;
    void* workspace = nullptr;
    uint64_t workspace_bytes = 0;
    void* radius_mem = nullptr;
    uint64_t radius_mem_bytes = 0;
    int num_cu = 0;
    void* bf_state_mem = nullptr;
    int64_t bf_state_rows = 0;
    int bf_knob[SLAM_BF_KNOBS] = {};
    int bf_engine = 0;
    void* bf_tbl_dev = nullptr;
    void* bf_tbl_host = nullptr;
    bool bf_tbl_ready = false;
    int bf_tbl_n[SLAM_BF_TBL_RING + 1] = {};
    bool bf_tbl_busy[SLAM_BF_TBL_RING + 1] = {};
    hipEvent_t bf_tbl_ev[SLAM_BF_TBL_RING] = {};
    int bf_tbl_cur = 0;
    void* scratch = nullptr;
    void* sel_host = nullptr;
    uint64_t sel_host_bytes = 0;
    std::vector<void*> sel_host_old;
    std::atomic<unsigned> done_epoch{0}, polled_calls{0};
    void* io_dev = nullptr;
    uint64_t io_dev_bytes = 0;
    void* io_host = nullptr;
    uint64_t io_host_bytes = 0;
    uint64_t io_h2d_bytes = 0, io_d2h_bytes = 0;
    int prof_on = 0;
    static const int PROF_MAX = 4096;
    hipEvent_t* prof_ev = nullptr;
    int prof_n = 0;
    void* comm = nullptr;
    int comm_rank = -1, comm_nranks = 0;
    hipStream_t comm_stream = nullptr;
    hipEvent_t comm_ready = nullptr;
    hipEvent_t comm_done[2] = {nullptr, nullptr};
    bool comm_done_valid[2] = {false, false};
};

int slam_set_error(int code, const char* fmt, ...);

#define SLAM_HIP(call)                                                              \
    do {                                                                            \
        hipError_t _e = (call);                                                     \
        if (_e != hipSuccess)                                                       \
            return slam_set_error(SLAM_ERR_HIP, "%s failed: %s (%s:%d)", #call,     \
                                  hipGetErrorString(_e), __FILE__, __LINE__);       \
    } while (0)

#define SLAM_REQUIRE(cond, ...)                                                     \
    do {                                                                            \
        if (!(cond)) return slam_set_error(SLAM_ERR_INVALID, __VA_ARGS__);          \
    } while (0)

int slam_workspace(slam_ctx* ctx, uint64_t bytes, void** out);
int slam_io_arena(slam_ctx* ctx, uint64_t dev_bytes, uint64_t host_bytes, void** dev, void** host);
static inline uint64_t slam_align_up(uint64_t v, uint64_t a = 256) { return (v + a - 1) / a * a; }
int slam_launch_check(const char* what);
int slam_occupancy_once(const void* kernel, std::atomic<int>* once, int* out);
struct bf_chunks {
    int qblocks, chunks;
    int64_t chunk;
};
bf_chunks bf_chunk_rule(int num_cu, int resident, int64_t N, int64_t rows, int64_t min_chunk, int64_t bytes_per_chunk,
                        int64_t cap_bytes);
int slam_bf_knn2_keep(slam_ctx* ctx, const void* d_query, int64_t N, const void* d_train, int64_t M, int64_t train_base,
                      int32_t* d_idx, int32_t* d_dist, void* d_keep);
int slam_bf_knn2_select(slam_ctx* ctx, const void* d_query, int64_t N, const void* d_train, int64_t M, int64_t train_base,
                        int32_t* d_idx, int32_t* d_dist, void* d_query_keep, int mode, double param, uint8_t* d_sel_keep,
                        int64_t* h_count);
int slam_bf_knn2_batch_keep(slam_ctx* ctx, int64_t B, const slam_bf_search* h_searches, void* const* h_keep, bool wait = false);
#define SLAM_BF_DONE_FLAGS 64
#define SLAM_BF_DONE_BYTES (SLAM_BF_DONE_FLAGS * 4)
int slam_done_block(slam_ctx* ctx, uint64_t extra);
unsigned slam_done_epoch(slam_ctx* ctx);
int slam_wait_done(slam_ctx* ctx, const unsigned* flags, int count, unsigned epoch);
#define SLAM_POSE_STAGE 512
int slam_pose_optimize_polled(slam_ctx* ctx, const double* d_pose_in, const double* d_points, const double* d_meas, int64_t O,
                              double fx, double fy, double cx, double cy, int rounds, int iterations, double chi2_threshold,
                              double huber_delta, double* d_pose_out, uint8_t* d_inlier, double* d_chi2, int32_t* d_stats,
                              unsigned* done, unsigned epoch);
int slam_filter_count(slam_ctx* ctx, const int32_t* d_idx, const int32_t* d_dist, int64_t N, int mode, double param,
                      uint8_t* d_keep, int64_t* h_count, int32_t* h_min_dist);
size_t bf_state_bytes(size_t rows);
int bf_state_reset(slam_ctx* ctx);
int slam_filter_launch(slam_ctx* ctx, const int32_t* d_idx, const int32_t* d_dist, int64_t N, int mode, double param,
                       uint8_t* d_keep, unsigned* done = nullptr, unsigned epoch = 0, bool* polled = nullptr);
int slam_cross_launch(slam_ctx* ctx, const int32_t* d_fwd_idx, const int32_t* d_fwd_dist, int64_t N,
                      const int32_t* d_rev_idx, int64_t M, int32_t* d_out_idx, int32_t* d_out_dist);
int slam_second_stream(slam_ctx* ctx);
void slam_second_stream_destroy(slam_ctx* ctx);
static inline unsigned int* slam_index_error_counter(slam_ctx* ctx) { return (unsigned int*)((char*)ctx->scratch + 1024); }
int slam_prof_begin(slam_ctx* ctx);
int slam_prof_end(slam_ctx* ctx);
```

### slam-experiments_amd/slamhip/__init__.py

```python
from ._lib import NO_MATCH_DIST, NO_MATCH_IDX, SlamHipBusy, SlamHipError, device_count, load
from .device import Context, DeviceBuffer, default_context, mx_plan_describe, mx_tile_describe, plan_describe
from .matching import (
    NORM_HAMMING,
    DeviceDescriptors,
    KeyframeDatabase,
    ResidentMatcher,
    Top2Table,
    as_descriptors,
    check_topk_k,
    cross_check_arrays,
    knn2_device,
    knn2_device_batch,
    knn2_select_device,
    knn_match_arrays,
    knn_match_arrays_batch,
    knn_match_collection,
    knn_topk_device,
    match_arrays,
    plan_describe_radius,
    plan_describe_topk,
    plan_describe_window,
    radius_device,
    radius_match_arrays,
    radius_match_collection,
    radius_threshold,
    ratio_test_arrays,
    split_image_index,
    topk_match_arrays,
    topk_match_collection,
    window_knn_device,
    window_match_arrays,
    window_match_filtered,
)
from .homography import (
    decompose_homography_arrays,
    decompose_homography_batch,
    decompose_homography_offsets,
    estimate_two_view_auto,
    find_homography_arrays,
    find_homography_batch,
    find_homography_offsets,
    fourpoint_homography_arrays,
    model_scores_offsets,
    verify_pairs_auto,
)
from .orb import (
    OrbExtractor,
    OrbFeatureDetector,
    OrbParams,
    OrbResult,
    orb_extract_arrays,
)
from .pnp import (
    loop_edges_from_pnp,
    p3p_arrays,
    solve_pnp_ransac,
    solve_pnp_ransac_batch,
    solve_pnp_ransac_offsets,
)
from .ba_sparse import SparseBAProblem, bundle_adjust_sparse, covisibility
from .covis import CovisibilityGraph, CovisibilityTables, covisibility_device
from .bow import (
    BowDatabase,
    BowVectors,
    Vocabulary,
    bow_transform,
    bow_vectors,
    detect_loop_candidates,
    read_dbow2_text,
    train_vocabulary,
    write_dbow2_text,
)
from .bow_match import (
    FeatureVectors,
    bow_feature_vectors,
    match_index_pairs,
    node_match_arrays,
    node_top2,
    search_by_bow,
    search_by_bow_descriptors,
)
from .proj_match import (
    FrameGrids,
    PointSets,
    proj_match_arrays,
    project_points,
    scale_tables,
    search_by_projection,
    search_by_sim3,
)
from .tri_match import (
    KeyframeViews,
    create_new_map_points,
    epi_match_arrays,
    epipole_in_second,
    fundamental_from_poses,
    search_for_triangulation,
    triangulate_matches,
)
from .fuse import (
    MapObservations,
    apply_fusion,
    fuse_arrays,
    fuse_by_sim3,
    fuse_points,
    refresh_map_points,
)
from .pose_graph import (
    loop_edges_from_two_view,
    optimize_pose_graph,
    pose_graph_hmul,
    pose_graph_linearize,
    pose_graph_pcg,
    read_g2o,
    write_g2o,
)
from .reproj import PoseOnlyProblem, ReprojProblem, build_linearization, poses_to_rt12
from .sim3 import (
    align_trajectory,
    estimate_sim3,
    estimate_sim3_batch,
    estimate_sim3_offsets,
    fit_sim3,
    fit_sim3_offsets,
    loop_edges_from_sim3,
    sim3_threepoint_arrays,
)
from .sim3_graph import (
    correct_points,
    lift_se3_graph,
    optimize_sim3_graph,
    sim3_edges_from_sim3,
    sim3_graph_hmul,
    sim3_graph_linearize,
    sim3_graph_pcg,
    sims_to_poses,
)
from .two_view import (
    estimate_two_view,
    find_essential_arrays,
    find_essential_batch,
    find_essential_offsets,
    fivepoint_arrays,
    mean_reprojection_error,
    recover_pose_arrays,
    recover_pose_batch,
    recover_pose_offsets,
    triangulate_arrays,
    verify_pairs,
)
```

### slam-experiments_amd/slamhip/_lib.py

```python
from __future__ import annotations

import ctypes
import os
from ctypes import POINTER, c_char_p, c_double, c_float, c_int, c_int32, c_int64, c_uint8, c_uint64, c_void_p

_HERE = os.path.dirname(os.path.abspath(__file__))
LIB_PATH = os.path.join(os.path.dirname(_HERE), "lib", "libslamhip.so")

SLAM_OK = 0
NO_MATCH_IDX = -1
NO_MATCH_DIST = 2**31 - 1
DESC_BYTES = 32
COMM_ID_BYTES = 128
P2P_HANDLE_BYTES = 64


class SlamHipError(RuntimeError):

    def __init__(self, code: int, message: str):
        super().__init__(f"libslamhip error {code}: {message}")
        self.code = code


class SlamHipBusy(SlamHipError):
    """SLAM_ERR_BUSY (-6): a resource condition, not a caller error - a kernel that needs all its workgroups resident at once
    could not get them (other work holds compute units).  Inputs and outputs are untouched; retry, or use the form without
    a residency requirement."""


SLAM_ERR_INVALID, SLAM_ERR_BUSY = -1, -6


SIGNATURES = {
    "slam_last_error": (c_char_p, []),
    "slam_version": (c_char_p, []),
    "slam_device_count": (c_int, [POINTER(c_int)]),
    "slam_ctx_create": (c_int, [c_int, POINTER(c_void_p)]),
    "slam_ctx_destroy": (c_int, [c_void_p]),
    "slam_ctx_device": (c_int, [c_void_p, POINTER(c_int)]),
    "slam_sync": (c_int, [c_void_p]),
    "slam_malloc": (c_int, [c_void_p, c_uint64, POINTER(c_void_p)]),
    "slam_free": (c_int, [c_void_p, c_void_p]),
    "slam_memset": (c_int, [c_void_p, c_void_p, c_int, c_uint64]),
    "slam_copy": (c_int, [c_void_p, c_void_p, c_void_p, c_uint64]),
    "slam_upload": (c_int, [c_void_p, c_void_p, c_void_p, c_uint64]),
    "slam_download": (c_int, [c_void_p, c_void_p, c_void_p, c_uint64]),
    "slam_timer_start": (c_int, [c_void_p]),
    "slam_timer_stop": (c_int, [c_void_p, POINTER(c_float)]),
    "slam_prof_enable": (c_int, [c_void_p, c_int]),
    "slam_prof_read": (c_int, [c_void_p, POINTER(c_int64), POINTER(c_double)]),
    "slam_bf_knn2_u256": (c_int, [c_void_p, c_void_p, c_int64, c_void_p, c_int64, c_int64, c_void_p, c_void_p]),
    "slam_bf_knn2_batch_u256": (c_int, [c_void_p, c_int64, c_void_p]),
    "slam_bf_knn2_select_u256": (c_int, [c_void_p, c_void_p, c_int64, c_void_p, c_int64, c_int64, c_void_p, c_void_p, c_int, c_double,
                                         c_void_p, POINTER(c_int64)]),
    "slam_bf_merge_top2": (c_int, [c_void_p, c_void_p, c_void_p, c_int64, c_int64, c_void_p, c_void_p]),
    "slam_bf_knn2_u256_host": (c_int, [c_void_p, c_void_p, c_int64, c_void_p, c_int64, c_void_p, c_void_p]),
    "slam_bf_knn_u256": (c_int, [c_void_p, c_void_p, c_int64, c_void_p, c_int64, c_int64, c_int, c_void_p, c_void_p]),
    "slam_bf_knn_u256_host": (c_int, [c_void_p, c_void_p, c_int64, c_void_p, c_int64, c_int, c_void_p, c_void_p]),
    "slam_bf_merge_topk": (c_int, [c_void_p, c_void_p, c_void_p, c_int64, c_int64, c_int, c_void_p, c_void_p]),
    "slam_bf_topk_plan_describe": (c_int, [c_int, c_int64, c_int64, c_int, POINTER(c_int32)]),
    "slam_bf_radius_u256": (c_int, [c_void_p, c_void_p, c_int64, c_void_p, c_int64, c_float, c_int64, c_void_p, c_int64, c_void_p,
                                    c_void_p, POINTER(c_int64)]),
    "slam_bf_radius_u256_host": (c_int, [c_void_p, c_void_p, c_int64, c_void_p, c_int64, c_float, c_void_p, c_int64, c_void_p,
                                         c_void_p, POINTER(c_int64)]),
    "slam_bf_radius_threshold": (c_int, [c_float]),
    "slam_bf_radius_plan_describe": (c_int, [c_int, c_int64, c_int64, POINTER(c_int32)]),
    "slam_bf_window_knn_u256": (c_int, [c_void_p, c_void_p, c_int64, c_void_p, c_int64, c_void_p, c_void_p, c_void_p, c_float,
                                        c_int, c_int64, c_void_p, c_void_p]),
    "slam_bf_window_knn_u256_host": (c_int, [c_void_p, c_void_p, c_int64, c_void_p, c_int64, c_void_p, c_void_p, c_void_p,
                                             c_float, c_int, c_int64, c_void_p, c_void_p]),
    "slam_bf_window_plan_describe": (c_int, [c_int, c_int64, c_int64, c_int64, POINTER(c_int64)]),
    "slam_bf_set_tuning": (c_int, [c_void_p, POINTER(c_int32), c_int]),
    "slam_bf_plan_info": (c_int, [c_void_p, c_int64, c_int64, POINTER(c_int32)]),
    "slam_bf_plan_describe": (c_int, [c_int, POINTER(c_int32), c_int, c_int64, c_int64, c_int64, c_int, POINTER(c_int32),
                                      POINTER(c_int32), c_int64, POINTER(c_int64)]),
    "slam_bf_set_engine": (c_int, [c_void_p, c_int]),
    "slam_bf_mx_plan_describe": (c_int, [c_int, c_int64, c_int64, POINTER(c_int32), POINTER(c_int32), c_int64, POINTER(c_int64)]),
    "slam_bf_mx_tile_describe": (c_int, [c_int, c_int64, c_int64, POINTER(c_int32)]),
    "slam_bf_reset_state": (c_int, [c_void_p]),
    "slam_bf_state_dirty": (c_int, [c_void_p, POINTER(c_int64)]),
    "slam_bf_match_filter": (c_int, [c_void_p, c_void_p, c_void_p, c_int64, c_int, c_double, c_void_p,
                                     POINTER(c_int64), POINTER(c_int32)]),
    "slam_bf_cross_check": (c_int, [c_void_p, c_void_p, c_void_p, c_int64, c_void_p, c_int64, c_void_p, c_void_p,
                                    POINTER(c_int64)]),
    "slam_bf_split_index": (c_int, [c_void_p, c_void_p, c_int64, c_void_p, c_int64, c_void_p, c_void_p]),
    "slam_reproj_rj_f64": (c_int, [c_void_p, c_void_p, c_int64, c_void_p, c_int64, c_void_p, c_void_p, c_void_p,
                                   c_int64, c_double, c_double, c_double, c_double, c_void_p, c_void_p, c_void_p]),
    "slam_pose_normal_eq_f64": (c_int, [c_void_p, c_void_p, c_void_p, c_void_p, c_void_p, c_int64, c_double,
                                        c_double, c_double, c_double, c_double, c_void_p, c_void_p, c_void_p]),
    "slam_pose_optimize_f64": (c_int, [c_void_p, c_void_p, c_void_p, c_void_p, c_int64, c_double, c_double, c_double,
                                       c_double, c_int, c_int, c_double, c_double, c_void_p, c_void_p, c_void_p,
                                       c_void_p]),
    "slam_pose_optimize_batch_f64": (c_int, [c_void_p, c_int64, c_void_p, c_void_p, c_void_p, c_void_p, c_int64, c_double,
                                             c_double, c_double, c_double, c_int, c_int, c_double, c_double, c_void_p,
                                             c_void_p, c_void_p, c_void_p]),
    "slam_tv_fivepoint_f64": (c_int, [c_void_p, c_int64, c_void_p, c_void_p, c_void_p, c_void_p]),
    "slam_tv_essential_ransac_f64": (c_int, [c_void_p, c_int64, c_void_p, c_void_p, c_void_p, c_int64, c_double, c_double, c_double,
                                             c_double, c_int, c_double, c_uint64, c_void_p, c_void_p, c_void_p]),
    "slam_tv_recover_pose_f64": (c_int, [c_void_p, c_int64, c_void_p, c_void_p, c_void_p, c_int64, c_double, c_double, c_double,
                                         c_double, c_void_p, c_void_p, c_double, c_void_p, c_void_p, c_void_p]),
    "slam_tv_triangulate_f64": (c_int, [c_void_p, c_int64, c_void_p, c_void_p, c_void_p, c_void_p, c_void_p, c_void_p]),
    "slam_pnp_p3p_f64": (c_int, [c_void_p, c_int64, c_void_p, c_void_p, c_void_p, c_void_p]),
    "slam_pnp_ransac_f64": (c_int, [c_void_p, c_int64, c_void_p, c_void_p, c_void_p, c_int64, c_double, c_double, c_double, c_double,
                                    c_int, c_double, c_uint64, c_void_p, c_void_p, c_void_p]),
    "slam_hg_fourpoint_f64": (c_int, [c_void_p, c_int64, c_void_p, c_void_p, c_void_p, c_void_p]),
    "slam_hg_ransac_f64": (c_int, [c_void_p, c_int64, c_void_p, c_void_p, c_void_p, c_int64, c_int, c_double, c_uint64, c_void_p,
                                   c_void_p, c_void_p]),
    "slam_hg_decompose_f64": (c_int, [c_void_p, c_int64, c_void_p, c_void_p, c_void_p, c_int64, c_double, c_double, c_double, c_double,
                                      c_void_p, c_void_p, c_double, c_void_p, c_void_p, c_void_p, c_void_p, c_void_p, c_void_p,
                                      c_void_p]),
    "slam_hg_model_score_f64": (c_int, [c_void_p, c_int64, c_void_p, c_void_p, c_void_p, c_int64, c_double, c_double, c_double,
                                        c_double, c_void_p, c_void_p, c_double, c_void_p, c_void_p]),
    "slam_sim3_threepoint_f64": (c_int, [c_void_p, c_int64, c_void_p, c_void_p, c_int, c_void_p, c_void_p]),
    "slam_sim3_ransac_f64": (c_int, [c_void_p, c_int64, c_void_p, c_void_p, c_void_p, c_int64, c_void_p, c_double, c_double, c_double,
                                     c_double, c_int, c_double, c_int, c_uint64, c_void_p, c_void_p, c_void_p]),
    "slam_sim3_refit_f64": (c_int, [c_void_p, c_int64, c_void_p, c_void_p, c_void_p, c_int64, c_void_p, c_int, c_void_p, c_void_p]),
    "slam_pg_workspace": (c_int, [c_int64, c_int64, POINTER(c_uint64)]),
    "slam_pg_plan": (c_int, [c_int64, c_int64, POINTER(c_int32)]),
    "slam_pg_linearize_f64": (c_int, [c_void_p, c_int64, c_int64, c_void_p, c_void_p, c_void_p, c_void_p, c_void_p, c_void_p,
                                      c_double, c_void_p, c_void_p, c_void_p, c_void_p, POINTER(c_int32)]),
    "slam_pg_hmul_f64": (c_int, [c_void_p, c_int64, c_int64, c_void_p, c_void_p, c_void_p, c_void_p, c_void_p, c_void_p,
                                 c_double, c_void_p, c_void_p]),
    "slam_pg_pcg_f64": (c_int, [c_void_p, c_int64, c_int64, c_void_p, c_void_p, c_void_p, c_void_p, c_void_p, c_void_p,
                                c_void_p, c_double, c_double, c_int, c_void_p, c_void_p]),
    "slam_pg_optimize_f64": (c_int, [c_void_p, c_int64, c_int64, c_void_p, c_void_p, c_void_p, c_void_p, c_void_p, c_int64,
                                     c_void_p, c_void_p, c_int, c_double, c_double, c_int, c_void_p, c_void_p]),
    "slam_pg_optimize_host_f64": (c_int, [c_void_p, c_int64, c_int64, c_void_p, c_void_p, c_void_p, c_void_p, c_void_p, c_int,
                                          c_double, c_double, c_int, c_void_p, c_void_p]),
    "slam_s3g_workspace": (c_int, [c_int64, c_int64, POINTER(c_uint64)]),
    "slam_s3g_plan": (c_int, [c_int64, c_int64, POINTER(c_int32)]),
    "slam_s3g_linearize_f64": (c_int, [c_void_p, c_int64, c_int64, c_void_p, c_void_p, c_void_p, c_void_p, c_void_p, c_void_p,
                                       c_double, c_void_p, c_void_p, c_void_p, c_void_p, POINTER(c_int32)]),
    "slam_s3g_hmul_f64": (c_int, [c_void_p, c_int64, c_int64, c_void_p, c_void_p, c_void_p, c_void_p, c_void_p, c_void_p,
                                  c_double, c_void_p, c_void_p]),
    "slam_s3g_pcg_f64": (c_int, [c_void_p, c_int64, c_int64, c_void_p, c_void_p, c_void_p, c_void_p, c_void_p, c_void_p,
                                 c_void_p, c_double, c_double, c_int, c_void_p, c_void_p]),
    "slam_s3g_optimize_f64": (c_int, [c_void_p, c_int64, c_int64, c_void_p, c_void_p, c_void_p, c_void_p, c_void_p, c_int64,
                                      c_void_p, c_void_p, c_int, c_double, c_double, c_int, c_int, c_void_p, c_void_p]),
    "slam_s3g_optimize_host_f64": (c_int, [c_void_p, c_int64, c_int64, c_void_p, c_void_p, c_void_p, c_void_p, c_void_p, c_int,
                                           c_double, c_double, c_int, c_int, c_void_p, c_void_p]),
    "slam_orb_workspace": (c_int, [c_int64, c_int64, c_int64, c_int, c_void_p, c_void_p, c_int64, POINTER(c_uint64), c_void_p]),
    "slam_orb_extract_u8": (c_int, [c_void_p, c_void_p, c_int64, c_int64, c_int64, c_void_p, c_int, c_int, c_void_p, c_void_p, c_void_p,
                                    c_int, c_void_p, c_void_p, c_uint64, c_void_p, c_void_p, c_void_p, c_void_p]),
    "slam_orb_extract_u8_host": (c_int, [c_void_p, c_void_p, c_int64, c_int64, c_int64, c_void_p, c_int, c_int, c_void_p, c_void_p,
                                         c_void_p, c_int, c_void_p, c_void_p, c_void_p, c_void_p, c_void_p]),
    "slam_bf_match_host": (c_int, [c_void_p, c_void_p, c_int64, c_void_p, c_void_p, c_int64, c_void_p, c_int, c_double,
                                   c_void_p, c_void_p, c_void_p, c_void_p]),
    "slam_index_errors": (c_int, [c_void_p, POINTER(c_int64)]),
    "slam_io_counters": (c_int, [c_void_p, POINTER(c_uint64), POINTER(c_uint64)]),
    "slam_ctx_block_bytes": (c_int, [c_void_p, POINTER(c_int64), c_int]),
    "slam_ctx_block_fill": (c_int, [c_void_p, c_int, c_int]),
    "slam_pose_optimize_host_f64": (c_int, [c_void_p, c_void_p, c_void_p, c_void_p, c_int64, c_double, c_double,
                                            c_double, c_double, c_int, c_int, c_double, c_double, c_void_p, c_void_p,
                                            c_void_p, c_void_p]),
    "slam_ba_reduce_f64": (c_int, [c_void_p, c_void_p, c_int64, c_void_p, c_int64, c_void_p, c_void_p, c_void_p,
                                   c_int64, c_void_p, c_void_p, c_void_p, c_void_p, c_void_p, c_double, c_double,
                                   c_double, c_double, c_double, c_double, c_void_p, c_void_p, c_void_p, c_void_p,
                                   c_void_p, c_void_p, c_void_p, c_void_p, c_void_p]),
    "slam_ba_cost_f64": (c_int, [c_void_p, c_void_p, c_int64, c_void_p, c_void_p, c_void_p, c_void_p, c_void_p, c_double,
                                 c_double, c_double, c_double, c_double, c_void_p]),
    "slam_ba_backsub_f64": (c_int, [c_void_p, c_int64, c_void_p, c_void_p, c_void_p, c_void_p, c_void_p, c_void_p,
                                    c_void_p, c_void_p]),
    "slam_ba_optimize_workspace": (c_int, [c_int64, c_int64, c_int64, POINTER(c_uint64)]),
    "slam_ba_optimize_shape": (c_int, [c_int64, c_int64, c_int64, POINTER(c_int32), POINTER(c_int32)]),
    "slam_ba_optimize_host_f64": (c_int, [c_void_p, c_int64, c_int64, c_int64, c_void_p, c_void_p, c_void_p, c_void_p, c_void_p,
                                          c_void_p, c_double, c_double, c_double, c_double, c_double, c_int, c_void_p, c_void_p,
                                          c_void_p]),
    "slam_ba_optimize_f64": (c_int, [c_void_p, c_int64, c_int64, c_int64, c_void_p, c_void_p, c_void_p, c_void_p, c_void_p, c_void_p,
                                     c_void_p, c_void_p, c_int64, c_double, c_double, c_double, c_double, c_double, c_int, c_void_p,
                                     c_void_p, c_void_p, c_uint64, c_void_p]),
    "slam_bas_workspace": (c_int, [c_int64, c_int64, c_int64, c_int64, c_int64, POINTER(c_uint64)]),
    "slam_bas_plan": (c_int, [c_int64, c_int64, c_int64, c_int64, c_int64, POINTER(c_int32)]),
    "slam_bas_linearize_f64": (c_int, [c_void_p, c_int64, c_int64, c_int64] + [c_void_p] * 10 + [c_double] * 5 + [c_void_p] * 7),
    "slam_bas_cost_f64": (c_int, [c_void_p, c_int64, c_int64, c_int64] + [c_void_p] * 7 + [c_double] * 5 + [c_void_p] * 2),
    "slam_bas_reduce_f64": (c_int, [c_void_p, c_int64, c_int64, c_int64, c_int64, c_int64] + [c_void_p] * 12 + [c_double] + [c_void_p] * 5),
    "slam_bas_backsub_f64": (c_int, [c_void_p, c_int64, c_int64, c_int64] + [c_void_p] * 8),
    "slam_bas_candidate_f64": (c_int, [c_void_p, c_int64, c_int64] + [c_void_p] * 7 + [c_double] + [c_void_p] * 4),
    "slam_bow_limits": (c_int, [POINTER(c_int32)]),
    "slam_bow_transform": (c_int, [c_void_p, c_void_p, c_int64, c_void_p, c_void_p, c_void_p, c_int64, c_int, c_int, c_int, c_void_p, c_void_p]),
    "slam_bow_vectors": (c_int, [c_void_p, c_void_p, c_void_p, c_int64, c_int64, c_void_p, c_int64, c_void_p, c_uint64, c_void_p,
                                 c_void_p, c_void_p, c_void_p]),
    "slam_bow_vectors_workspace": (c_int, [c_int64, c_int64, POINTER(c_uint64)]),
    "slam_bow_group_keys": (c_int, [c_void_p, c_void_p, c_int64, c_int64, c_void_p, c_void_p, c_void_p]),
    "slam_bow_index_build": (c_int, [c_void_p, c_void_p, c_void_p, c_void_p, c_int64, c_int64, c_void_p, c_void_p, c_void_p, c_void_p]),
    "slam_bow_query": (c_int, [c_void_p, c_void_p, c_void_p, c_void_p, c_int64, c_void_p, c_void_p, c_int64, c_int64, c_int64, c_int,
                               c_void_p, c_void_p, c_void_p, c_void_p, c_void_p]),
    "slam_bow_train_seed": (c_int, [c_void_p, c_void_p, c_int64, c_void_p, c_int64, c_int, c_void_p, c_void_p, c_void_p, c_uint64]),
    "slam_bow_train_seed_workspace": (c_int, [c_int64, c_int64, POINTER(c_uint64)]),
    "slam_bow_train_step": (c_int, [c_void_p, c_void_p, c_int64, c_void_p, c_int64, c_int, c_void_p, c_void_p, c_void_p, c_void_p, c_int64,
                                    c_void_p, c_void_p, c_void_p, c_int, POINTER(c_int64)]),
    "slam_bow_train_descend": (c_int, [c_void_p, c_void_p, c_void_p, c_int64, c_int64, c_int, c_void_p, c_void_p]),
    "slam_bow_match_limits": (c_int, [POINTER(c_int32)]),
    "slam_bow_match_plan_describe": (c_int, [c_int64, c_int64, POINTER(c_int64)]),
    "slam_bow_match_group": (c_int, [c_void_p, c_void_p, c_void_p, c_void_p, c_int64, c_void_p, c_void_p, c_void_p, c_void_p]),
    "slam_bow_match_top2": (c_int, [c_void_p, c_void_p, c_void_p, c_void_p, c_int64, c_int, c_void_p, c_void_p]),
    "slam_bow_match_search": (c_int, [c_void_p, c_void_p, c_void_p, c_void_p, c_int64, c_int, c_double, c_int, c_void_p, c_void_p,
                                      c_void_p, c_void_p]),
    "slam_proj_match_limits": (c_int, [POINTER(c_int32)]),
    "slam_proj_match_plan_describe": (c_int, [c_int64, c_int64, c_int64, POINTER(c_int64)]),
    "slam_proj_match_grid": (c_int, [c_void_p, c_void_p, c_void_p, c_void_p, c_void_p, c_void_p, c_int64, c_int, c_int, c_int, c_void_p,
                                     c_void_p, c_void_p, c_void_p, c_void_p, c_void_p, c_void_p]),
    "slam_proj_match_project": (c_int, [c_void_p, c_void_p, c_void_p, c_void_p, c_void_p, c_void_p, c_int64, c_void_p, c_void_p, c_void_p,
                                        c_void_p, c_void_p]),
    "slam_proj_match_search": (c_int, [c_void_p, c_void_p, c_void_p, c_void_p, c_void_p, c_void_p, c_void_p, c_int64, c_void_p, c_void_p,
                                       c_void_p, c_void_p, c_void_p, c_void_p, c_void_p, c_void_p, c_void_p]),
    "slam_tri_match_limits": (c_int, [POINTER(c_int32)]),
    "slam_tri_match_plan_describe": (c_int, [c_int64, c_int64, POINTER(c_int64)]),
    "slam_tri_match_search": (c_int, [c_void_p, c_void_p, c_void_p, c_void_p, c_void_p, c_void_p, c_int64, c_void_p, c_void_p, c_void_p,
                                      c_int, c_void_p, c_void_p, c_void_p, c_void_p]),
    "slam_tri_match_triangulate": (c_int, [c_void_p, c_void_p, c_int64, c_void_p, c_int64, c_void_p, c_void_p, c_void_p, c_int64,
                                           c_void_p, c_void_p, c_void_p, c_void_p, c_void_p, c_void_p, c_void_p, c_void_p, c_void_p,
                                           c_void_p, c_void_p]),
    "slam_fuse_limits": (c_int, [POINTER(c_int32)]),
    "slam_fuse_search": (c_int, [c_void_p] * 8 + [c_int64] + [c_void_p] * 4 + [c_int64] + [c_void_p] * 10),
    "slam_fuse_refresh": (c_int, [c_void_p, c_void_p, c_void_p, c_void_p, c_int64, c_void_p, c_int64, c_void_p, c_void_p, c_void_p,
                                  c_void_p, c_int64, c_void_p, c_void_p, c_void_p, c_int] + [c_void_p] * 4),
    "slam_covis_limits": (c_int, [POINTER(c_int32)]),
    "slam_covis_plan": (c_int, [c_int64, c_int64, c_int64, c_int64, POINTER(c_int32)]),
    "slam_covis_workspace": (c_int, [c_int64, c_int64, c_int64, c_int64, POINTER(c_uint64)]),
    "slam_covis_count": (c_int, [c_void_p, c_int64, c_int64, c_int64, c_void_p, c_void_p, c_void_p, c_void_p, POINTER(c_int64)]),
    "slam_covis_pairs": (c_int, [c_void_p, c_int64, c_int64, c_int64, c_int64, c_void_p, c_void_p, c_void_p, c_void_p, POINTER(c_int64)]),
    "slam_covis_edges": (c_int, [c_void_p, c_int64, c_int64, c_int64, c_void_p, c_void_p, c_void_p, c_void_p]),
    "slam_covis_rows": (c_int, [c_void_p, c_int64, c_int64, c_void_p, c_void_p, c_void_p, c_void_p]),
    "slam_comm_version": (c_int, [POINTER(c_int)]),
    "slam_comm_unique_id": (c_int, [c_void_p]),
    "slam_comm_init": (c_int, [c_void_p, c_int, c_int, c_void_p]),
    "slam_comm_destroy": (c_int, [c_void_p]),
    "slam_comm_allgather": (c_int, [c_void_p, c_void_p, c_void_p, c_uint64]),
    "slam_comm_broadcast": (c_int, [c_void_p, c_void_p, c_uint64, c_int]),
    "slam_comm_allgather_overlapped": (c_int, [c_void_p, c_void_p, c_void_p, c_uint64, c_int]),
    "slam_comm_wait_buffer": (c_int, [c_void_p, c_int]),
    "slam_p2p_export": (c_int, [c_void_p, c_void_p, c_void_p]),
    "slam_p2p_open": (c_int, [c_void_p, c_void_p, POINTER(c_void_p)]),
    "slam_p2p_close": (c_int, [c_void_p, c_void_p]),
    "slam_p2p_allgather_overlapped": (c_int, [c_void_p, c_void_p, c_uint64, c_int, c_void_p, c_int, c_int]),
}

class BfSearch(ctypes.Structure):

    _fields_ = [("d_query", c_void_p), ("N", c_int64), ("d_train", c_void_p), ("M", c_int64), ("train_base", c_int64),
                ("d_idx", c_void_p), ("d_dist", c_void_p)]


class BowGroups(ctypes.Structure):

    _fields_ = [("d_desc", c_void_p), ("d_nodes", c_void_p), ("d_order", c_void_p), ("d_inverse", c_void_p), ("d_bins", c_void_p),
                ("h_offsets", c_void_p), ("B", c_int64)]


class ProjFrames(ctypes.Structure):

    _fields_ = [("d_desc", c_void_p), ("d_cells", c_void_p), ("d_order", c_void_p), ("d_xy", c_void_p), ("d_meta", c_void_p),
                ("d_level", c_void_p), ("d_bins", c_void_p), ("h_offsets", c_void_p), ("B", c_int64), ("W", c_int32), ("H", c_int32),
                ("cell", c_int32), ("pad", c_int32)]


class ProjPoints(ctypes.Structure):

    _fields_ = [("d_xyz", c_void_p), ("d_desc", c_void_p), ("d_range", c_void_p), ("d_normal", c_void_p), ("d_level", c_void_p),
                ("d_bins", c_void_p), ("h_offsets", c_void_p), ("B", c_int64)]


class ProjParams(ctypes.Structure):

    _fields_ = [("fx", c_double), ("fy", c_double), ("cx", c_double), ("cy", c_double), ("min_x", c_double), ("max_x", c_double),
                ("min_y", c_double), ("max_y", c_double), ("cos2_limit", c_double), ("ratio", c_double), ("h_scale", c_void_p),
                ("h_scale2", c_void_p), ("n_levels", c_int32), ("th_high", c_int32), ("level_rule", c_int32), ("lo", c_int32), ("hi", c_int32),
                ("pad", c_int32)]


class TriViews(ctypes.Structure):

    _fields_ = [("d_xy", c_void_p), ("d_level", c_void_p), ("d_taken", c_void_p)]


class TriParams(ctypes.Structure):

    _fields_ = [("fx", c_double), ("fy", c_double), ("cx", c_double), ("cy", c_double), ("chi2", c_double), ("epipole_r2", c_double),
                ("cos_max", c_double), ("chi2_px", c_double), ("ratio_factor", c_double), ("h_scale", c_void_p), ("h_sigma2", c_void_p),
                ("n_levels", c_int32), ("th_low", c_int32)]


class FuseParams(ctypes.Structure):

    _fields_ = [("m_lo2", c_double), ("m_hi2", c_double), ("chi2", c_double), ("th_low", c_int32), ("pad", c_int32)]


BF_BATCH_MAX = 32
BF_KNN_MAX = 32
_lib = None


def load() -> ctypes.CDLL:
    global _lib
    if _lib is not None:
        return _lib
    if not os.path.exists(LIB_PATH):
        raise ImportError(
            f"{LIB_PATH} is missing: build it with `python -c 'import __graft_entry__ as g; g.build()'` "
            "(make -C slam-experiments_amd/csrc). There is no CPU fallback."
        )
    lib = ctypes.CDLL(LIB_PATH, mode=ctypes.RTLD_GLOBAL)
    for name, (res, args) in SIGNATURES.items():
        fn = getattr(lib, name)
        fn.restype = res
        fn.argtypes = args
    _lib = lib
    return lib


def addr(a) -> int:
    try:
        return ctypes.addressof(ctypes.c_char.from_buffer(a))
    except (TypeError, ValueError):
        return a.__array_interface__["data"][0]


def check(rc: int) -> None:
    if rc != SLAM_OK:
        msg = load().slam_last_error()
        raise (SlamHipBusy if rc == SLAM_ERR_BUSY else SlamHipError)(rc, msg.decode("utf-8", "replace") if msg else "unknown error")


def device_count() -> int:
    n = c_int(0)
    rc = load().slam_device_count(ctypes.byref(n))
    return n.value if rc == SLAM_OK else 0
```

### slam-experiments_amd/slamhip/device.py

```python
from __future__ import annotations

import ctypes
import threading
from typing import Optional, Tuple

import numpy as np

from . import _lib
from ._lib import check


class DeviceBuffer:

    __slots__ = ("ctx", "ptr", "nbytes", "_owner")

    def __init__(self, ctx: "Context", ptr: int, nbytes: int, owner: Optional["DeviceBuffer"] = None):
        self.ctx = ctx
        self.ptr = ptr
        self.nbytes = nbytes
        self._owner = owner

    def view(self, offset: int, nbytes: Optional[int] = None) -> "DeviceBuffer":
        nbytes = self.nbytes - offset if nbytes is None else nbytes
        if offset < 0 or nbytes < 0 or offset + nbytes > self.nbytes:
            raise ValueError("view out of range")
        return DeviceBuffer(self.ctx, self.ptr + offset, nbytes, self._owner or self)

    def upload(self, host: np.ndarray) -> "DeviceBuffer":
        host = np.ascontiguousarray(host)
        if host.nbytes > self.nbytes:
            raise ValueError(f"upload of {host.nbytes} B into a {self.nbytes} B buffer")
        check(self.ctx.lib.slam_upload(self.ctx.handle, self.ptr, host.ctypes.data, host.nbytes))
        return self

    def download(self, dtype, shape) -> np.ndarray:
        out = np.empty(shape, dtype)
        if out.nbytes > self.nbytes:
            raise ValueError(f"download of {out.nbytes} B from a {self.nbytes} B buffer")
        check(self.ctx.lib.slam_download(self.ctx.handle, out.ctypes.data, self.ptr, out.nbytes))
        return out

    def free(self) -> None:
        if self._owner is None and self.ptr:
            check(self.ctx.lib.slam_free(self.ctx.handle, self.ptr))
            self.ptr = 0


class Context:

    def __init__(self, device: int = 0):
        self.lib = _lib.load()
        h = ctypes.c_void_p()
        check(self.lib.slam_ctx_create(device, ctypes.byref(h)))
        self.handle = h
        self.device = device

    def close(self) -> None:
        if self.handle:
            check(self.lib.slam_ctx_destroy(self.handle))
            self.handle = None

    def __enter__(self):
        return self

    def __exit__(self, *exc):
        self.close()

    def malloc(self, nbytes: int) -> DeviceBuffer:
        p = ctypes.c_void_p()
        check(self.lib.slam_malloc(self.handle, int(nbytes), ctypes.byref(p)))
        return DeviceBuffer(self, p.value or 0, int(nbytes))

    def upload(self, host: np.ndarray) -> DeviceBuffer:
        host = np.ascontiguousarray(host)
        return self.malloc(host.nbytes).upload(host)

    def set_tuning(self, R: int = 0, blocks_per_cu: int = 0, lead_rows: int = 0, lead_chunk: int = 0,
                   tail: int = 0, feed: int = 0, cold: int = 0, chunk: int = 0, queue: int = 0, merge: int = 0) -> None:
        knobs = (ctypes.c_int32 * 10)(R, blocks_per_cu, lead_rows, lead_chunk, tail, feed, cold, chunk, queue, merge)
        check(self.lib.slam_bf_set_tuning(self.handle, knobs, 10))

    def set_engine(self, engine: int = 0) -> None:
        check(self.lib.slam_bf_set_engine(self.handle, int(engine)))

    def state_dirty(self) -> int:
        n = ctypes.c_int64(-1)
        check(self.lib.slam_bf_state_dirty(self.handle, ctypes.byref(n)))
        return n.value

    BLOCKS = ("workspace", "merge_state", "pinned_block", "io_dev", "io_host", "radius_tables")

    def block_bytes(self) -> dict:
        b = (ctypes.c_int64 * len(self.BLOCKS))()
        check(self.lib.slam_ctx_block_bytes(self.handle, b, len(self.BLOCKS)))
        return dict(zip(self.BLOCKS, b))

    def fill_block(self, name: str, byte: int) -> None:
        check(self.lib.slam_ctx_block_fill(self.handle, self.BLOCKS.index(name), int(byte) & 0xFF))

    def plan_info(self, n: int, m: int) -> dict:
        p = (ctypes.c_int32 * 10)()
        check(self.lib.slam_bf_plan_info(self.handle, n, m, p))
        return dict(zip(("R", "qblocks", "chunk", "chunks", "lead_rows", "lead_chunks", "tail_chunks", "cus", "sgpr_feed", "cold_rows"), p))

    def sync(self) -> None:
        check(self.lib.slam_sync(self.handle))

    def timer_start(self) -> None:
        check(self.lib.slam_timer_start(self.handle))

    def timer_stop(self) -> float:
        ms = ctypes.c_float(0)
        check(self.lib.slam_timer_stop(self.handle, ctypes.byref(ms)))
        return ms.value

    def prof_enable(self, on: bool = True) -> None:
        check(self.lib.slam_prof_enable(self.handle, int(on)))

    def prof_read(self) -> Tuple[int, float]:
        n = ctypes.c_int64(0)
        ms = ctypes.c_double(0)
        check(self.lib.slam_prof_read(self.handle, ctypes.byref(n), ctypes.byref(ms)))
        return n.value, ms.value


_default_lock = threading.Lock()
_default_ctx: Optional[Context] = None


def default_context() -> Context:
    global _default_ctx
    with _default_lock:
        if _default_ctx is None:
            _default_ctx = Context(0)
        return _default_ctx


PLAN_KNOBS = ("R", "blocks_per_cu", "lead_rows", "lead_chunk", "tail", "feed", "cold", "chunk", "queue", "merge")


def mx_plan_describe(n: int, m: int, num_cu: int = 256):
    lib = _lib.load()
    plan = (ctypes.c_int32 * 8)()
    cap = 1 << 16
    tbl = (ctypes.c_int32 * cap)()
    length = ctypes.c_int64(0)
    check(lib.slam_bf_mx_plan_describe(num_cu, n, m, plan, tbl, cap, ctypes.byref(length)))
    names = ("qblocks", "workers", "chunk", "chunks", "tail_chunks", "stage_rows", "resident", "auto")
    return dict(zip(names, plan)), list(tbl[:min(length.value, cap)])


def mx_tile_describe(n: int, m: int, engine: int = 0) -> int:
    tile = ctypes.c_int32(0)
    check(_lib.load().slam_bf_mx_tile_describe(int(engine), n, m, ctypes.byref(tile)))
    return tile.value


def plan_describe(n: int, m: int, num_cu: int = 256, qb_all: int = 0, rows_on_host: bool = False, **knobs):
    unknown = set(knobs) - set(PLAN_KNOBS)
    if unknown:
        raise TypeError(f"unknown knobs {sorted(unknown)}")
    lib = _lib.load()
    k = (ctypes.c_int32 * len(PLAN_KNOBS))(*(int(knobs.get(name, 0)) for name in PLAN_KNOBS))
    plan = (ctypes.c_int32 * 14)()
    cap = 1 << 16
    tbl = (ctypes.c_int32 * cap)()
    length = ctypes.c_int64(0)
    check(lib.slam_bf_plan_describe(num_cu, k, len(PLAN_KNOBS), n, m, qb_all, int(rows_on_host), plan, tbl, cap, ctypes.byref(length)))
    names = ("R", "qblocks", "chunk", "chunks", "lead_rows", "lead_chunks", "tail_chunks", "cus", "sgpr_feed", "cold_rows",
             "table_free", "bound_free", "workers", "resident")
    out = dict(zip(names, plan))
    out["merge"], out["resident"] = out["resident"] >> 8, out["resident"] & 255
    return out, list(tbl[:min(length.value, cap)])
```

Before: 12050 billion.

## Pre-expand train descriptors into an MX image and stream it directly into LDS

```diff
diff --git a/include/slamhip.h b/include/slamhip.h
--- a/include/slamhip.h
+++ b/include/slamhip.h
@@ -107,6 +107,10 @@
 SLAM_API int slam_bf_mx_plan_describe(int num_cu, int64_t N, int64_t M, int32_t* h_plan, int32_t* h_tbl, int64_t tbl_cap,
                                       int64_t* tbl_len);
 SLAM_API int slam_bf_mx_tile_describe(int engine, int64_t N, int64_t M, int32_t* h_tile);
+SLAM_API int slam_bf_set_mx_feed(slam_ctx* ctx, int feed);
+SLAM_API int slam_bf_mx_feed_describe(int feed, int64_t N, int64_t M, int32_t* h_feed);
+SLAM_API int slam_bf_mx_image_bytes(slam_ctx* ctx, int64_t* h_bytes);
+SLAM_API int slam_bf_mx_image_fill(slam_ctx* ctx, int byte);
 SLAM_API int slam_bf_reset_state(slam_ctx* ctx);
 SLAM_API int slam_bf_state_dirty(slam_ctx* ctx, int64_t* h_words);
 
diff --git a/slam-experiments_amd/csrc/bf_mx.hip b/slam-experiments_amd/csrc/bf_mx.hip
--- a/slam-experiments_amd/csrc/bf_mx.hip
+++ b/slam-experiments_amd/csrc/bf_mx.hip
@@ -338,6 +338,57 @@
     return SLAM_OK;
 }
 
+static bool bf_mx_feed_auto(int64_t N, int64_t M) {
+    return N >= 65536 && N <= 131072 && M >= 65536 && M <= 200000;
+}
+
+extern "C" int slam_bf_mx_feed_describe(int feed, int64_t N, int64_t M, int32_t* h_feed) {
+    SLAM_REQUIRE(h_feed, "slam_bf_mx_feed_describe: null argument");
+    SLAM_REQUIRE(feed >= 0 && feed <= 2, "feed must be 0 (auto), 1 (expand in the kernel) or 2 (prepared image)");
+    SLAM_REQUIRE(N >= 1 && M >= 1, "bad sizes");
+    *h_feed = feed == 2 || (feed == 0 && bf_mx_feed_auto(N, M)) ? 2 : 1;
+    return SLAM_OK;
+}
+
+extern "C" int slam_bf_set_mx_feed(slam_ctx* ctx, int feed) {
+    SLAM_REQUIRE(ctx, "slam_bf_set_mx_feed: null ctx");
+    SLAM_REQUIRE(feed >= 0 && feed <= 2, "feed must be 0 (auto), 1 (expand in the kernel) or 2 (prepared image)");
+    std::lock_guard<std::mutex> g(ctx->mu);
+    ctx->bf_mx_feed = feed;
+    return SLAM_OK;
+}
+
+static int bf_mx_image_get(slam_ctx* ctx, uint64_t bytes, void** out) {
+    if (bytes > ctx->bf_mx_img_bytes) {
+        SLAM_HIP(hipStreamSynchronize(ctx->stream));
+        if (ctx->bf_mx_img) SLAM_HIP(hipFree(ctx->bf_mx_img));
+        ctx->bf_mx_img = nullptr;
+        ctx->bf_mx_img_bytes = 0;
+        const uint64_t want = bytes + (bytes >> 2);
+        SLAM_HIP(hipMalloc(&ctx->bf_mx_img, want));
+        ctx->bf_mx_img_bytes = want;
+    }
+    *out = ctx->bf_mx_img;
+    return SLAM_OK;
+}
+
+extern "C" int slam_bf_mx_image_bytes(slam_ctx* ctx, int64_t* h_bytes) {
+    SLAM_REQUIRE(ctx && h_bytes, "slam_bf_mx_image_bytes: null argument");
+    std::lock_guard<std::mutex> lk(ctx->call_mu);
+    *h_bytes = (int64_t)ctx->bf_mx_img_bytes;
+    return SLAM_OK;
+}
+extern "C" int slam_bf_mx_image_fill(slam_ctx* ctx, int byte) {
+    SLAM_REQUIRE(ctx, "slam_bf_mx_image_fill: null ctx");
+    std::lock_guard<std::mutex> lk(ctx->call_mu);
+    SLAM_HIP(hipSetDevice(ctx->device));
+    SLAM_HIP(hipStreamSynchronize(ctx->stream));
+    if (!ctx->bf_mx_img || !ctx->bf_mx_img_bytes) return SLAM_OK;
+    SLAM_HIP(hipMemsetAsync(ctx->bf_mx_img, byte, ctx->bf_mx_img_bytes, ctx->stream));
+    SLAM_HIP(hipStreamSynchronize(ctx->stream));
+    return SLAM_OK;
+}
+
 extern "C" int slam_bf_set_engine(slam_ctx* ctx, int engine) {
     SLAM_REQUIRE(ctx, "slam_bf_set_engine: null ctx");
     SLAM_REQUIRE(engine >= 0 && engine <= 3,
@@ -357,21 +408,24 @@
 
 int bf_mx_pass(slam_ctx* ctx, const void* d_query, int64_t N, const void* d_train, int64_t M, int64_t train_base, int32_t* d_idx,
                int32_t* d_dist, void* d_keep, const bf_select& sel, int* qblocks_out) {
-    int num_cu, engine;
+    int num_cu, engine, feed;
     {
         std::lock_guard<std::mutex> g(ctx->mu);
         num_cu = ctx->num_cu;
         engine = ctx->bf_engine;
+        feed = ctx->bf_mx_feed;
     }
     const bool wide = engine == 3 || (engine == 0 && bf_mx32_auto(N, M));
-    const auto kernel = wide ? bf_top2_mx32_kernel : bf_top2_mx_kernel;
-    static std::atomic<int> occ_once[2] = {{0}, {0}};
-    int occ = occ_once[wide].load(std::memory_order_relaxed);
+    const bool image = wide && (feed == 2 || (feed == 0 && bf_mx_feed_auto(N, M)));
+    const auto kernel = image ? bf_mx32_image_top2_kernel : wide ? bf_top2_mx32_kernel : bf_top2_mx_kernel;
+    const int which = image ? 2 : wide ? 1 : 0;
+    static std::atomic<int> occ_once[3] = {{0}, {0}, {0}};
+    int occ = occ_once[which].load(std::memory_order_relaxed);
     if (!occ) {
         int o = 0;
         SLAM_HIP(hipOccupancyMaxActiveBlocksPerMultiprocessor(&o, kernel, 256, 0));
         occ = o > 0 ? o : SLAM_MX_RESIDENT;
-        occ_once[wide].store(occ, std::memory_order_relaxed);
+        occ_once[which].store(occ, std::memory_order_relaxed);
     }
     std::vector<int> tbl;
     const bf_mx_plan p = make_mx_plan_core(num_cu, occ, N, M, &tbl);
@@ -381,9 +435,21 @@
     if (int rc = bf_table_get(ctx, tbl, &d_tbl)) return rc;
     if (qblocks_out) *qblocks_out = p.qblocks;
     SLAM_HIP(hipGetLastError());
+    const void* d_rows = d_train;
+    if (image) {
+        for (size_t i = 0; i + 1 < tbl.size(); i++)
+            SLAM_REQUIRE(tbl[i] % SLAM_MX_STAGE == 0, "MX plan: chunk %zu starts at row %d, not a multiple of the stage", i, tbl[i]);
+        const int64_t rows = (M + SLAM_MX_STAGE - 1) / SLAM_MX_STAGE * SLAM_MX_STAGE;
+        void* img = nullptr;
+        if (int rc = bf_mx_image_get(ctx, (uint64_t)rows * SLAM_MX_IMAGE_ROW_BYTES, &img)) return rc;
+        bf_mx_image_kernel<<<dim3((unsigned)(rows * 2 / 256)), dim3(256), 0, ctx->stream>>>((const u32*)d_train, (int)M, (uint4*)img,
+                                                                                            (int)rows);
+        if (int rc = slam_launch_check("train image kernel")) return rc;
+        d_rows = img;
+    }
     if (int rc = slam_prof_begin(ctx)) return rc;
     kernel<<<dim3(p.qblocks, p.workers), dim3(256), 0, ctx->stream>>>(
-        (const uint4*)d_query, (int)N, (const uint4*)d_train, d_tbl, st, (int)train_base, (int2*)d_idx, (int2*)d_dist,
+        (const uint4*)d_query, (int)N, (const uint4*)d_rows, d_tbl, st, (int)train_base, (int2*)d_idx, (int2*)d_dist,
         (uint4*)d_keep, p.S, sel);
     if (int rc = slam_prof_end(ctx)) return rc;
     const hipError_t e = hipGetLastError();
diff --git a/slam-experiments_amd/csrc/bf_mx32.hip b/slam-experiments_amd/csrc/bf_mx32.hip
--- a/slam-experiments_amd/csrc/bf_mx32.hip
+++ b/slam-experiments_amd/csrc/bf_mx32.hip
@@ -22,228 +22,41 @@
 #define MX32_GROUP 32
 #define MX32_GROUPS (SLAM_MX_STAGE / MX32_GROUP)
 
-__global__ __launch_bounds__(256) __attribute__((amdgpu_waves_per_eu(4, 4))) void bf_top2_mx32_kernel(
-    const uint4* __restrict__ q, int N, const uint4* __restrict__ t, const int* __restrict__ tbl, bf_state st, int train_base,
-    int2* __restrict__ out_idx, int2* __restrict__ out_dist, uint4* __restrict__ keep, int nchunks, bf_select sel) {
-    __shared__ uint4 tile[2][SLAM_MX_STAGE * 8];
-    __shared__ u32 s_ticket, s_last;
-    const int tid = threadIdx.x;
-    const int lane = tid & 63, wave = tid >> 6;
-    const int hk = lane >> 5, col = lane & 31;
-#ifdef SLAM_MX_PROBE
-    unsigned long long pacc[8] = {0, 0, 0, 0, 0, 0, 0, 0}, plast = __builtin_readcyclecounter();
-#endif
-    const int bx = ((int)blockIdx.x + (int)blockIdx.y) % (int)gridDim.x;
-    auto lane_query = [&]() -> int {
-        int v = tid;
-        asm volatile("" : "+v"(v));
-        return bx * 256 + v;
-    };
+__device__ __forceinline__ void mx32_copy_stage(const uint4* src, u32 voff, u32 lds) {
+    const char* p = (const char*)src;
+    u32 keep;
+    asm volatile(
+        "s_mov_b32 %0, m0\n\t"
+        "s_mov_b32 m0, %6\n\ts_nop 0\n\tglobal_load_lds_dwordx4 %1, %2\n\t"
+        "s_add_u32 m0, m0, 0x1000\n\ts_nop 0\n\tglobal_load_lds_dwordx4 %1, %3\n\t"
+        "s_add_u32 m0, m0, 0x1000\n\ts_nop 0\n\tglobal_load_lds_dwordx4 %1, %4\n\t"
+        "s_add_u32 m0, m0, 0x1000\n\ts_nop 0\n\tglobal_load_lds_dwordx4 %1, %5\n\t"
+        "s_mov_b32 m0, %0"
+        : "=&s"(keep)
+        : "v"(voff), "s"(p), "s"(p + 4096), "s"(p + 8192), "s"(p + 12288), "s"(lds)
+        : "memory", "scc");
+}
+__device__ __forceinline__ void mx32_copies_done() { asm volatile("s_waitcnt vmcnt(0)" ::: "memory"); }
 
-    uint4 qb[2][4];
-    const u32* qw = (const u32*)q;
-#pragma unroll
-    for (int tt = 0; tt < 2; tt++) {
-        int qi = bx * 256 + wave * 64 + tt * 32 + col;
-        qi = qi < N ? qi : N - 1;
-#pragma unroll
-        for (int kq = 0; kq < 4; kq++) qb[tt][kq] = mx_expand(qw[(size_t)qi * 8 + kq * 2 + hk]);
-    }
-    if (const int qbase = lane_query(); keep && blockIdx.y == 0 && qbase < N) {
-        keep[2 * (size_t)qbase] = q[2 * (size_t)qbase];
-        keep[2 * (size_t)qbase + 1] = q[2 * (size_t)qbase + 1];
-    }
+#define MX32_KERNEL bf_top2_mx32_kernel
+#define MX32_IMAGE_FEED 0
+#include "bf_mx32_scan.inc"
+#undef MX32_KERNEL
+#undef MX32_IMAGE_FEED
+#define MX32_KERNEL bf_mx32_image_top2_kernel
+#define MX32_IMAGE_FEED 1
+#include "bf_mx32_scan.inc"
+#undef MX32_KERNEL
+#undef MX32_IMAGE_FEED
 
-    u32 b1[2], b2[2], xs[2];
-    int thr[2];
-    auto set_threshold = [&](int tt, u32 x) {
-        xs[tt] = x;
-        thr[tt] = x > 129u ? (int)0x80000000u : __float_as_int((float)(258 - 2 * (int)x));
-    };
-#pragma unroll
-    for (int tt = 0; tt < 2; tt++) {
-        b1[tt] = b2[tt] = SLAM_KEY_NONE;
-        set_threshold(tt, SLAM_KEY_NONE >> SLAM_KEY_IDX_BITS);
-    }
-    auto unite_tile = [&](int tt, u32& u1, u32& u2) {
-        u1 = b1[tt];
-        u2 = b2[tt];
-        const u32 c1 = (u32)__shfl_xor((int)u1, 32, 64), c2 = (u32)__shfl_xor((int)u2, 32, 64);
-        mx_unite(u1, u2, c1, c2);
-    };
-    u32 gkey = SLAM_BOUND_IDLE, pend[1] = {0u};
-    auto exchange = [&](int c0) {
-        u32 u1[2], u2[2];
-#pragma unroll
-        for (int tt = 0; tt < 2; tt++) unite_tile(tt, u1[tt], u2[tt]);
-        if (const int qbase = lane_query(); qbase < N) {
-            const u32 own = hk ? u2[1] : u2[0];
-            asm volatile("" ::"v"(pend[0]));
-            const u32 g = __hip_atomic_load(&st.bound[qbase], __ATOMIC_RELAXED, __HIP_MEMORY_SCOPE_AGENT);
-            if (own < g && own < SLAM_MX_BOUND_LIMIT) pend[0] = atomicMin(&st.bound[qbase], own);
-            gkey = g;
-        }
-#pragma unroll
-        for (int tt = 0; tt < 2; tt++) {
-            const u32 g = (u32)__shfl((int)gkey, tt * 32 + col, 64);
-            set_threshold(tt, min(xs[tt], min(mx_bound_x(g, c0), u2[tt] >> SLAM_KEY_IDX_BITS)));
-        }
-    };
-
-    const int srow = tid >> 1, sh = tid & 1;
-    auto load_stage = [&](int s, int c1) -> uint4 {
-        const uint4* ts = t + 2 * (size_t)s;
-        if (s + SLAM_MX_STAGE <= c1) return ts[(u32)tid];
-        return s + srow < c1 ? ts[(u32)tid] : make_uint4(0, 0, 0, 0);
-    };
-    const u32 fill = 0x22222222u;
-    uint4* const dst0 = tile[0] + (srow >> 5) * 256 + sh * 128 + (srow & 31);
-    auto store_word = [&](uint4* dst, int j, u32 v) { dst[(j >> 1) * 64 + (j & 1) * 32] = mx_expand_op(v, fill); };
-    auto store_stage = [&](int b, uint4 v) {
-        uint4* dst = dst0 + b * (SLAM_MX_STAGE * 8);
-        store_word(dst, 0, v.x);
-        store_word(dst, 1, v.y);
-        store_word(dst, 2, v.z);
-        store_word(dst, 3, v.w);
-    };
-
-    u32* const cursor = st.cursor + (size_t)(4 * bx) * SLAM_CURSOR_STRIDE;
-    if (tid == 0) s_ticket = __hip_atomic_fetch_add(cursor, 1u, __ATOMIC_RELAXED, __HIP_MEMORY_SCOPE_AGENT);
-    __syncthreads();
-    int ci = __builtin_amdgcn_readfirstlane((int)s_ticket);
-    int scanned = 0;
-    MX_STAMP(0);
-    while (ci < nchunks) {
-        const int c0 = tbl[ci], c1 = tbl[ci + 1];
-        const uint4 first = load_stage(c0, c1);
-        exchange(c0);
-        store_stage(0, first);
-        __syncthreads();
-        MX_STAMP(1);
-        int buf = 0;
-        for (int s0 = c0; s0 < c1; s0 += SLAM_MX_STAGE) {
-            const int s1 = s0 + SLAM_MX_STAGE;
-            const bool more = s1 < c1;
-            if (!more && tid == 0) s_ticket = __hip_atomic_fetch_add(cursor, 1u, __ATOMIC_RELAXED, __HIP_MEMORY_SCOPE_AGENT);
-            MX_STAMP(7);
-            const uint4* tp = tile[buf];
-            auto fold_tile = [&](int tt, int g, const mx_v16f& acc, auto rag) {
-                int p = max(max(__float_as_int(acc[0]), __float_as_int(acc[1])), __float_as_int(acc[2]));
-#pragma unroll
-                for (int i = 3; i < 15; i += 2) p = max(max(p, __float_as_int(acc[i])), __float_as_int(acc[i + 1]));
-                const int m = max(p, __float_as_int(acc[15]));
-                if (__builtin_expect(__ballot(m >= thr[tt]) == 0ull, 1)) return;
-                MX_STAMP(2);
-                int row0 = s0 + g * MX32_GROUP;
-                asm("" : "+s"(row0));
-                const u32 rowk = (u32)row0 + (u32)(4 * hk);
-                const u32 base = (128u << SLAM_KEY_IDX_BITS) + rowk;
-                unsigned long long gate[16];
-#pragma unroll
-                for (int i = 0; i < 16; i++) gate[i] = __ballot(__float_as_int(acc[i]) >= thr[tt]);
-                asm volatile("" ::"s"(gate[0]), "s"(gate[1]), "s"(gate[2]), "s"(gate[3]), "s"(gate[4]), "s"(gate[5]), "s"(gate[6]),
-                             "s"(gate[7]), "s"(gate[8]), "s"(gate[9]), "s"(gate[10]), "s"(gate[11]), "s"(gate[12]), "s"(gate[13]),
-                             "s"(gate[14]), "s"(gate[15]));
-#pragma unroll
-                for (int i = 0; i < 16; i++) {
-                    if (gate[i] == 0ull) continue;
-                    const int off = 8 * (i >> 2) + (i & 3);
-                    u32 key = base + (u32)off + ((u32)(int)(-acc[i]) << (SLAM_KEY_IDX_BITS - 1));
-                    if constexpr (decltype(rag)::value)
-                        key = (int)rowk + off < c1 ? key : SLAM_KEY_NONE;
-                    b2[tt] = umed3(b1[tt], b2[tt], key);
-                    b1[tt] = min(b1[tt], key);
-                }
-                set_threshold(tt, min(xs[tt], b2[tt] >> SLAM_KEY_IDX_BITS));
-                MX_STAMP(3);
-            };
-            const mx_v16f zero = {0, 0, 0, 0, 0, 0, 0, 0, 0, 0, 0, 0, 0, 0, 0, 0};
-            auto group = [&](int g, auto rag) {
-                mx_v16f acc[2];
-#pragma unroll
-                for (int kq = 0; kq < 4; kq++) {
-                    const uint4 a = tp[g * 256 + kq * 64 + lane];
-#pragma unroll
-                    for (int tt = 0; tt < 2; tt++) acc[tt] = mx32_dot(a, qb[tt][kq], kq ? acc[tt] : zero);
-                }
-#pragma unroll
-                for (int tt = 0; tt < 2; tt++) fold_tile(tt, g, acc[tt], rag);
-            };
-            auto trip = [&](auto shadow) {
-                constexpr bool SH = decltype(shadow)::value;
-                const uint4* ap = tp + lane;
-                uint4* const dst = dst0 + (buf ^ 1) * (SLAM_MX_STAGE * 8);
-                u32 nx[4] = {0, 0, 0, 0};
-                if (SH) {
-                    const uint4 x = (t + 2 * (size_t)s1)[2 * min(srow, c1 - 1 - s1) + sh];
-                    nx[0] = x.x; nx[1] = x.y; nx[2] = x.z; nx[3] = x.w;
-                }
-                uint4 a[4];
-#pragma unroll
-                for (int kq = 0; kq < 4; kq++) a[kq] = ap[kq * 64];
-                mx_v16f acc[2];
-                auto dot = [&](int tt, int kq) {
-                    __builtin_amdgcn_sched_barrier(0);
-                    acc[tt] = mx32_dot(a[kq], qb[tt][kq], kq ? acc[tt] : zero);
-                    __builtin_amdgcn_sched_barrier(0);
-                };
-#pragma unroll
-                for (int k = 0; k < MX32_GROUPS; k++) {
-                    auto ahead = [&](int kq) {
-                        if (k + 1 < MX32_GROUPS) a[kq] = ap[(k + 1) * 256 + kq * 64];
-                        __builtin_amdgcn_sched_barrier(0);
-                    };
-                    dot(0, 0);
-                    dot(0, 1);
-                    dot(0, 2);
-                    dot(0, 3);
-                    if (k) fold_tile(1, k - 1, acc[1], std::false_type{});
-                    dot(1, 0);
-                    ahead(0);
-                    dot(1, 1);
-                    ahead(1);
-                    if (SH && k >= 1) store_word(dst, k - 1, nx[k - 1]);
-                    dot(1, 2);
-                    ahead(2);
-                    if (SH && k == 3) store_word(dst, 3, nx[3]);
-                    dot(1, 3);
-                    ahead(3);
-                    fold_tile(0, k, acc[0], std::false_type{});
-                }
-                __builtin_amdgcn_sched_barrier(0);
-                fold_tile(1, MX32_GROUPS - 1, acc[1], std::false_type{});
-            };
-            if (more) {
-                trip(std::true_type{});
-            } else if (s1 == c1) {
-                trip(std::false_type{});
-            } else {
-                const int ng = __builtin_amdgcn_readfirstlane((c1 - s0 + MX32_GROUP - 1) / MX32_GROUP);
-                for (int g = 0; g < ng; g++) group(g, std::true_type{});
-            }
-            MX_STAMP(2);
-            scanned += min(s1, c1) - s0;
-            if (more && scanned < 32 * SLAM_MX_STAGE && (SLAM_MX_EARLY >> (scanned / SLAM_MX_STAGE) & 1u)) exchange(s1);
-            MX_STAMP(4);
-            __syncthreads();
-            MX_STAMP(5);
-            buf ^= 1;
-        }
-        ci = __builtin_amdgcn_readfirstlane((int)s_ticket);
-    }
-
-    u32 u1[2], u2[2];
-#pragma unroll
-    for (int tt = 0; tt < 2; tt++) unite_tile(tt, u1[tt], u2[tt]);
-    const u32 f1[1] = {hk ? u1[1] : u1[0]}, f2[1] = {hk ? u2[1] : u2[0]};
-    const u32 gk[1] = {gkey < SLAM_MX_BOUND_LIMIT ? gkey >> SLAM_KEY_IDX_BITS : SLAM_BOUND_IDLE};
-    bf_top2_epilogue<1, true>(st, bx, tid, lane, lane_query(), false, false, f1, f2, gk, pend, N, (int)gridDim.y, train_base, out_idx,
-                              out_dist, sel, s_last);
-#ifdef SLAM_MX_PROBE
-    MX_STAMP(6);
-    if (g_mx32_probe && lane == 0) {
-        unsigned long long* o = g_mx32_probe + ((size_t)(blockIdx.y * gridDim.x + blockIdx.x) * 4 + wave) * 8;
-        for (int i = 0; i < 8; i++) o[i] = pacc[i];
-    }
-#endif
+__global__ __launch_bounds__(256) void bf_mx_image_kernel(const u32* __restrict__ t, int M, uint4* __restrict__ img, int rows) {
+    const int i = (int)(blockIdx.x * 256 + threadIdx.x);
+    const int row = i >> 1, sh = i & 1;
+    if (row >= rows) return;
+    const uint4 v = row < M ? ((const uint4*)t)[i] : make_uint4(0, 0, 0, 0);
+    uint4* dst = img + (size_t)(row >> 5) * 256 + sh * 128 + (row & 31);
+    dst[0] = mx_expand(v.x);
+    dst[32] = mx_expand(v.y);
+    dst[64] = mx_expand(v.z);
+    dst[96] = mx_expand(v.w);
 }
diff --git a/slam-experiments_amd/csrc/bf_mx32_scan.inc b/slam-experiments_amd/csrc/bf_mx32_scan.inc
--- /dev/null
+++ b/slam-experiments_amd/csrc/bf_mx32_scan.inc
@@ -0,0 +1,239 @@
+__global__ __launch_bounds__(256) __attribute__((amdgpu_waves_per_eu(4, 4))) void MX32_KERNEL(
+    const uint4* __restrict__ q, int N, const uint4* __restrict__ t, const int* __restrict__ tbl, bf_state st, int train_base,
+    int2* __restrict__ out_idx, int2* __restrict__ out_dist, uint4* __restrict__ keep, int nchunks, bf_select sel) {
+    constexpr bool IMG = MX32_IMAGE_FEED;
+    __shared__ uint4 tile[2][SLAM_MX_STAGE * 8];
+    __shared__ u32 s_ticket, s_last;
+    const int tid = threadIdx.x;
+    const int lane = tid & 63, wave = tid >> 6;
+    const int hk = lane >> 5, col = lane & 31;
+#ifdef SLAM_MX_PROBE
+    unsigned long long pacc[8] = {0, 0, 0, 0, 0, 0, 0, 0}, plast = __builtin_readcyclecounter();
+#endif
+    const int bx = ((int)blockIdx.x + (int)blockIdx.y) % (int)gridDim.x;
+    auto lane_query = [&]() -> int {
+        int v = tid;
+        asm volatile("" : "+v"(v));
+        return bx * 256 + v;
+    };
+
+    uint4 qb[2][4];
+    const u32* qw = (const u32*)q;
+#pragma unroll
+    for (int tt = 0; tt < 2; tt++) {
+        int qi = bx * 256 + wave * 64 + tt * 32 + col;
+        qi = qi < N ? qi : N - 1;
+#pragma unroll
+        for (int kq = 0; kq < 4; kq++) qb[tt][kq] = mx_expand(qw[(size_t)qi * 8 + kq * 2 + hk]);
+    }
+    if (const int qbase = lane_query(); keep && blockIdx.y == 0 && qbase < N) {
+        keep[2 * (size_t)qbase] = q[2 * (size_t)qbase];
+        keep[2 * (size_t)qbase + 1] = q[2 * (size_t)qbase + 1];
+    }
+
+    u32 b1[2], b2[2], xs[2];
+    int thr[2];
+    auto set_threshold = [&](int tt, u32 x) {
+        xs[tt] = x;
+        thr[tt] = x > 129u ? (int)0x80000000u : __float_as_int((float)(258 - 2 * (int)x));
+    };
+#pragma unroll
+    for (int tt = 0; tt < 2; tt++) {
+        b1[tt] = b2[tt] = SLAM_KEY_NONE;
+        set_threshold(tt, SLAM_KEY_NONE >> SLAM_KEY_IDX_BITS);
+    }
+    auto unite_tile = [&](int tt, u32& u1, u32& u2) {
+        u1 = b1[tt];
+        u2 = b2[tt];
+        const u32 c1 = (u32)__shfl_xor((int)u1, 32, 64), c2 = (u32)__shfl_xor((int)u2, 32, 64);
+        mx_unite(u1, u2, c1, c2);
+    };
+    u32 gkey = SLAM_BOUND_IDLE, pend[1] = {0u};
+    auto exchange = [&](int c0) {
+        u32 u1[2], u2[2];
+#pragma unroll
+        for (int tt = 0; tt < 2; tt++) unite_tile(tt, u1[tt], u2[tt]);
+        if (const int qbase = lane_query(); qbase < N) {
+            const u32 own = hk ? u2[1] : u2[0];
+            asm volatile("" ::"v"(pend[0]));
+            const u32 g = __hip_atomic_load(&st.bound[qbase], __ATOMIC_RELAXED, __HIP_MEMORY_SCOPE_AGENT);
+            if (own < g && own < SLAM_MX_BOUND_LIMIT) pend[0] = atomicMin(&st.bound[qbase], own);
+            gkey = g;
+        }
+#pragma unroll
+        for (int tt = 0; tt < 2; tt++) {
+            const u32 g = (u32)__shfl((int)gkey, tt * 32 + col, 64);
+            set_threshold(tt, min(xs[tt], min(mx_bound_x(g, c0), u2[tt] >> SLAM_KEY_IDX_BITS)));
+        }
+    };
+
+    const int srow = tid >> 1, sh = tid & 1;
+    auto load_stage = [&](int s, int c1) -> uint4 {
+        const uint4* ts = t + 2 * (size_t)s;
+        if (s + SLAM_MX_STAGE <= c1) return ts[(u32)tid];
+        return s + srow < c1 ? ts[(u32)tid] : make_uint4(0, 0, 0, 0);
+    };
+    const u32 fill = 0x22222222u;
+    uint4* const dst0 = tile[0] + (srow >> 5) * 256 + sh * 128 + (srow & 31);
+    auto store_word = [&](uint4* dst, int j, u32 v) { dst[(j >> 1) * 64 + (j & 1) * 32] = mx_expand_op(v, fill); };
+    auto store_stage = [&](int b, uint4 v) {
+        uint4* dst = dst0 + b * (SLAM_MX_STAGE * 8);
+        store_word(dst, 0, v.x);
+        store_word(dst, 1, v.y);
+        store_word(dst, 2, v.z);
+        store_word(dst, 3, v.w);
+    };
+    auto copy_stage = [&](int b, int s) {
+        const u32 lds = (u32)(size_t)(__attribute__((address_space(3))) void*)(tile[b] + __builtin_amdgcn_readfirstlane(wave) * 64);
+        mx32_copy_stage(t + (size_t)s * 8, (u32)tid * 16u, lds);
+    };
+
+    u32* const cursor = st.cursor + (size_t)(4 * bx) * SLAM_CURSOR_STRIDE;
+    if (tid == 0) s_ticket = __hip_atomic_fetch_add(cursor, 1u, __ATOMIC_RELAXED, __HIP_MEMORY_SCOPE_AGENT);
+    __syncthreads();
+    int ci = __builtin_amdgcn_readfirstlane((int)s_ticket);
+    int scanned = 0;
+    MX_STAMP(0);
+    while (ci < nchunks) {
+        const int c0 = tbl[ci], c1 = tbl[ci + 1];
+        if constexpr (IMG) {
+            copy_stage(0, c0);
+            exchange(c0);
+            mx32_copies_done();
+        } else {
+            const uint4 first = load_stage(c0, c1);
+            exchange(c0);
+            store_stage(0, first);
+        }
+        __syncthreads();
+        MX_STAMP(1);
+        int buf = 0;
+        for (int s0 = c0; s0 < c1; s0 += SLAM_MX_STAGE) {
+            const int s1 = s0 + SLAM_MX_STAGE;
+            const bool more = s1 < c1;
+            if (!more && tid == 0) s_ticket = __hip_atomic_fetch_add(cursor, 1u, __ATOMIC_RELAXED, __HIP_MEMORY_SCOPE_AGENT);
+            MX_STAMP(7);
+            const uint4* tp = tile[buf];
+            auto fold_tile = [&](int tt, int g, const mx_v16f& acc, auto rag) {
+                int p = max(max(__float_as_int(acc[0]), __float_as_int(acc[1])), __float_as_int(acc[2]));
+#pragma unroll
+                for (int i = 3; i < 15; i += 2) p = max(max(p, __float_as_int(acc[i])), __float_as_int(acc[i + 1]));
+                const int m = max(p, __float_as_int(acc[15]));
+                if (__builtin_expect(__ballot(m >= thr[tt]) == 0ull, 1)) return;
+                MX_STAMP(2);
+                int row0 = s0 + g * MX32_GROUP;
+                asm("" : "+s"(row0));
+                const u32 rowk = (u32)row0 + (u32)(4 * hk);
+                const u32 base = (128u << SLAM_KEY_IDX_BITS) + rowk;
+                unsigned long long gate[16];
+#pragma unroll
+                for (int i = 0; i < 16; i++) gate[i] = __ballot(__float_as_int(acc[i]) >= thr[tt]);
+                asm volatile("" ::"s"(gate[0]), "s"(gate[1]), "s"(gate[2]), "s"(gate[3]), "s"(gate[4]), "s"(gate[5]), "s"(gate[6]),
+                             "s"(gate[7]), "s"(gate[8]), "s"(gate[9]), "s"(gate[10]), "s"(gate[11]), "s"(gate[12]), "s"(gate[13]),
+                             "s"(gate[14]), "s"(gate[15]));
+#pragma unroll
+                for (int i = 0; i < 16; i++) {
+                    if (gate[i] == 0ull) continue;
+                    const int off = 8 * (i >> 2) + (i & 3);
+                    u32 key = base + (u32)off + ((u32)(int)(-acc[i]) << (SLAM_KEY_IDX_BITS - 1));
+                    if constexpr (decltype(rag)::value)
+                        key = (int)rowk + off < c1 ? key : SLAM_KEY_NONE;
+                    b2[tt] = umed3(b1[tt], b2[tt], key);
+                    b1[tt] = min(b1[tt], key);
+                }
+                set_threshold(tt, min(xs[tt], b2[tt] >> SLAM_KEY_IDX_BITS));
+                MX_STAMP(3);
+            };
+            const mx_v16f zero = {0, 0, 0, 0, 0, 0, 0, 0, 0, 0, 0, 0, 0, 0, 0, 0};
+            auto group = [&](int g, auto rag) {
+                mx_v16f acc[2];
+#pragma unroll
+                for (int kq = 0; kq < 4; kq++) {
+                    const uint4 a = tp[g * 256 + kq * 64 + lane];
+#pragma unroll
+                    for (int tt = 0; tt < 2; tt++) acc[tt] = mx32_dot(a, qb[tt][kq], kq ? acc[tt] : zero);
+                }
+#pragma unroll
+                for (int tt = 0; tt < 2; tt++) fold_tile(tt, g, acc[tt], rag);
+            };
+            auto trip = [&](auto shadow) {
+                constexpr bool SH = decltype(shadow)::value;
+                const uint4* ap = tp + lane;
+                uint4* const dst = dst0 + (buf ^ 1) * (SLAM_MX_STAGE * 8);
+                u32 nx[4] = {0, 0, 0, 0};
+                if constexpr (SH && IMG) {
+                    copy_stage(buf ^ 1, s1);
+                } else if (SH) {
+                    const uint4 x = (t + 2 * (size_t)s1)[2 * min(srow, c1 - 1 - s1) + sh];
+                    nx[0] = x.x; nx[1] = x.y; nx[2] = x.z; nx[3] = x.w;
+                }
+                uint4 a[4];
+#pragma unroll
+                for (int kq = 0; kq < 4; kq++) a[kq] = ap[kq * 64];
+                mx_v16f acc[2];
+                auto dot = [&](int tt, int kq) {
+                    __builtin_amdgcn_sched_barrier(0);
+                    acc[tt] = mx32_dot(a[kq], qb[tt][kq], kq ? acc[tt] : zero);
+                    __builtin_amdgcn_sched_barrier(0);
+                };
+#pragma unroll
+                for (int k = 0; k < MX32_GROUPS; k++) {
+                    auto ahead = [&](int kq) {
+                        if (k + 1 < MX32_GROUPS) a[kq] = ap[(k + 1) * 256 + kq * 64];
+                        __builtin_amdgcn_sched_barrier(0);
+                    };
+                    dot(0, 0);
+                    dot(0, 1);
+                    dot(0, 2);
+                    dot(0, 3);
+                    if (k) fold_tile(1, k - 1, acc[1], std::false_type{});
+                    dot(1, 0);
+                    ahead(0);
+                    dot(1, 1);
+                    ahead(1);
+                    if (SH && !IMG && k >= 1) store_word(dst, k - 1, nx[k - 1]);
+                    dot(1, 2);
+                    ahead(2);
+                    if (SH && !IMG && k == 3) store_word(dst, 3, nx[3]);
+                    dot(1, 3);
+                    ahead(3);
+                    fold_tile(0, k, acc[0], std::false_type{});
+                }
+                __builtin_amdgcn_sched_barrier(0);
+                fold_tile(1, MX32_GROUPS - 1, acc[1], std::false_type{});
+            };
+            if (more) {
+                trip(std::true_type{});
+            } else if (s1 == c1) {
+                trip(std::false_type{});
+            } else {
+                const int ng = __builtin_amdgcn_readfirstlane((c1 - s0 + MX32_GROUP - 1) / MX32_GROUP);
+                for (int g = 0; g < ng; g++) group(g, std::true_type{});
+            }
+            MX_STAMP(2);
+            scanned += min(s1, c1) - s0;
+            if (more && scanned < 32 * SLAM_MX_STAGE && (SLAM_MX_EARLY >> (scanned / SLAM_MX_STAGE) & 1u)) exchange(s1);
+            MX_STAMP(4);
+            if constexpr (IMG) mx32_copies_done();
+            __syncthreads();
+            MX_STAMP(5);
+            buf ^= 1;
+        }
+        ci = __builtin_amdgcn_readfirstlane((int)s_ticket);
+    }
+
+    u32 u1[2], u2[2];
+#pragma unroll
+    for (int tt = 0; tt < 2; tt++) unite_tile(tt, u1[tt], u2[tt]);
+    const u32 f1[1] = {hk ? u1[1] : u1[0]}, f2[1] = {hk ? u2[1] : u2[0]};
+    const u32 gk[1] = {gkey < SLAM_MX_BOUND_LIMIT ? gkey >> SLAM_KEY_IDX_BITS : SLAM_BOUND_IDLE};
+    bf_top2_epilogue<1, true>(st, bx, tid, lane, lane_query(), false, false, f1, f2, gk, pend, N, (int)gridDim.y, train_base, out_idx,
+                              out_dist, sel, s_last);
+#ifdef SLAM_MX_PROBE
+    MX_STAMP(6);
+    if (g_mx32_probe && lane == 0) {
+        unsigned long long* o = g_mx32_probe + ((size_t)(blockIdx.y * gridDim.x + blockIdx.x) * 4 + wave) * 8;
+        for (int i = 0; i < 8; i++) o[i] = pacc[i];
+    }
+#endif
+}
diff --git a/slam-experiments_amd/csrc/bf_mx_common.h b/slam-experiments_amd/csrc/bf_mx_common.h
--- a/slam-experiments_amd/csrc/bf_mx_common.h
+++ b/slam-experiments_amd/csrc/bf_mx_common.h
@@ -47,3 +47,8 @@
 __global__ void bf_top2_mx32_kernel(const uint4* __restrict__ q, int N, const uint4* __restrict__ t, const int* __restrict__ tbl,
                                     bf_state st, int train_base, int2* __restrict__ out_idx, int2* __restrict__ out_dist,
                                     uint4* __restrict__ keep, int nchunks, bf_select sel);
+__global__ void bf_mx32_image_top2_kernel(const uint4* __restrict__ q, int N, const uint4* __restrict__ t, const int* __restrict__ tbl,
+                                          bf_state st, int train_base, int2* __restrict__ out_idx, int2* __restrict__ out_dist,
+                                          uint4* __restrict__ keep, int nchunks, bf_select sel);
+__global__ void bf_mx_image_kernel(const u32* __restrict__ t, int M, uint4* __restrict__ img, int rows);
+#define SLAM_MX_IMAGE_ROW_BYTES 128
diff --git a/slam-experiments_amd/csrc/ctx.hip b/slam-experiments_amd/csrc/ctx.hip
--- a/slam-experiments_amd/csrc/ctx.hip
+++ b/slam-experiments_amd/csrc/ctx.hip
@@ -74,6 +74,7 @@
     if (ctx->sel_host) (void)hipHostFree(ctx->sel_host);
     for (void* old : ctx->sel_host_old) (void)hipHostFree(old);
     if (ctx->bf_state_mem) (void)hipFree(ctx->bf_state_mem);
+    if (ctx->bf_mx_img) (void)hipFree(ctx->bf_mx_img);
     if (ctx->bf_tbl_ready) {
         (void)hipFree(ctx->bf_tbl_dev);
         (void)hipHostFree(ctx->bf_tbl_host);
diff --git a/slam-experiments_amd/csrc/internal.h b/slam-experiments_amd/csrc/internal.h
--- a/slam-experiments_amd/csrc/internal.h
+++ b/slam-experiments_amd/csrc/internal.h
@@ -28,6 +28,9 @@
     int64_t bf_state_rows = 0;
     int bf_knob[SLAM_BF_KNOBS] = {};
     int bf_engine = 0;
+    int bf_mx_feed = 0;
+    void* bf_mx_img = nullptr;
+    uint64_t bf_mx_img_bytes = 0;
     void* bf_tbl_dev = nullptr;
     void* bf_tbl_host = nullptr;
     bool bf_tbl_ready = false;
diff --git a/slam-experiments_amd/slamhip/__init__.py b/slam-experiments_amd/slamhip/__init__.py
--- a/slam-experiments_amd/slamhip/__init__.py
+++ b/slam-experiments_amd/slamhip/__init__.py
@@ -1,5 +1,5 @@
 from ._lib import NO_MATCH_DIST, NO_MATCH_IDX, SlamHipBusy, SlamHipError, device_count, load
-from .device import Context, DeviceBuffer, default_context, mx_plan_describe, mx_tile_describe, plan_describe
+from .device import Context, DeviceBuffer, default_context, mx_feed_describe, mx_plan_describe, mx_tile_describe, plan_describe
 from .matching import (
     NORM_HAMMING,
     DeviceDescriptors,
diff --git a/slam-experiments_amd/slamhip/_lib.py b/slam-experiments_amd/slamhip/_lib.py
--- a/slam-experiments_amd/slamhip/_lib.py
+++ b/slam-experiments_amd/slamhip/_lib.py
@@ -77,6 +77,10 @@
     "slam_bf_set_engine": (c_int, [c_void_p, c_int]),
     "slam_bf_mx_plan_describe": (c_int, [c_int, c_int64, c_int64, POINTER(c_int32), POINTER(c_int32), c_int64, POINTER(c_int64)]),
     "slam_bf_mx_tile_describe": (c_int, [c_int, c_int64, c_int64, POINTER(c_int32)]),
+    "slam_bf_set_mx_feed": (c_int, [c_void_p, c_int]),
+    "slam_bf_mx_feed_describe": (c_int, [c_int, c_int64, c_int64, POINTER(c_int32)]),
+    "slam_bf_mx_image_bytes": (c_int, [c_void_p, POINTER(c_int64)]),
+    "slam_bf_mx_image_fill": (c_int, [c_void_p, c_int]),
     "slam_bf_reset_state": (c_int, [c_void_p]),
     "slam_bf_state_dirty": (c_int, [c_void_p, POINTER(c_int64)]),
     "slam_bf_match_filter": (c_int, [c_void_p, c_void_p, c_void_p, c_int64, c_int, c_double, c_void_p,
diff --git a/slam-experiments_amd/slamhip/device.py b/slam-experiments_amd/slamhip/device.py
--- a/slam-experiments_amd/slamhip/device.py
+++ b/slam-experiments_amd/slamhip/device.py
@@ -83,6 +83,17 @@
     def set_engine(self, engine: int = 0) -> None:
         check(self.lib.slam_bf_set_engine(self.handle, int(engine)))
 
+    def set_mx_feed(self, feed: int = 0) -> None:
+        check(self.lib.slam_bf_set_mx_feed(self.handle, int(feed)))
+
+    def mx_image_bytes(self) -> int:
+        n = ctypes.c_int64(-1)
+        check(self.lib.slam_bf_mx_image_bytes(self.handle, ctypes.byref(n)))
+        return n.value
+
+    def fill_mx_image(self, byte: int) -> None:
+        check(self.lib.slam_bf_mx_image_fill(self.handle, int(byte) & 0xFF))
+
     def state_dirty(self) -> int:
         n = ctypes.c_int64(-1)
         check(self.lib.slam_bf_state_dirty(self.handle, ctypes.byref(n)))
@@ -156,6 +167,12 @@
     return tile.value
 
 
+def mx_feed_describe(n: int, m: int, feed: int = 0) -> int:
+    out = ctypes.c_int32(0)
+    check(_lib.load().slam_bf_mx_feed_describe(int(feed), n, m, ctypes.byref(out)))
+    return out.value
+
+
 def plan_describe(n: int, m: int, num_cu: int = 256, qb_all: int = 0, rows_on_host: bool = False, **knobs):
     unknown = set(knobs) - set(PLAN_KNOBS)
     if unknown:
```

Result: faster. 12180 billion (median of 6 runs) (+1.1%).
